# DonggeunYu/Text2Speech

Measured on AMD Instinct MI355X. Metric: WaveGlow forward audio samples/sec (batch 8x16000 per GPU), higher is better.
Workload: dtype bf16x3 (split-bf16 products, f32 accumulate); 1 GPU; WaveGlow forward, batch 8 x 16000 samples per GPU, 12 flows, n_group 8, WN 8 layers x 512 channels (reference waveglow/config.json); per_gpu_batch=8, segment_length=16000, mode=forward, parallelism=replicas, no collective

## Files before the change

### include/t2s_hip.h

```cpp
#ifndef T2S_HIP_H
#define T2S_HIP_H
#include <stddef.h>
#ifdef __cplusplus
extern "C" {
#endif

#define T2S_OK 0
#define T2S_EINVAL (-1)
#define T2S_EHIP (-2)

#define T2S_PERM_NONE 0
#define T2S_PERM_GATE 1
#define T2S_PERM_PAIR8 2
#define T2S_ACT_NONE 0
#define T2S_ACT_RELU 1
#define T2S_ACT_TANH 2

int t2s_abi_version(void);
int t2s_operand_format(void);
int t2s_sizeof_taco_decoder(void);
int t2s_sizeof_taco_bptt(void);
const char* t2s_error_string(int code);
const char* t2s_last_hip_error(void);

int t2s_plane_rows(int L, int halo);
int t2s_padded_rows(int rows);

int t2s_pack_conv_weight(const float* v, const float* g, int g_is_scale, const float* bias_in, int O, int Cin, int Kt,
                         int perm, int C_gate, int row_off, int Mpad, int koff, int Cin_pad, void* A_hi, void* A_lo,
                         float* bias_out, int bias_accumulate, void* stream);

typedef struct t2s_pack_job {
    const float *v, *g, *bias_in, *bias_in2;
    void *A_hi, *A_lo;
    float* bias_out;
    long row_start;
    long O, Cin, Kt, perm, C_gate, Mpad, koff, Cin_pad, row_off, g_is_scale;
    float* scale_out;
} t2s_pack_job;
int t2s_pack_conv_weight_table(const t2s_pack_job* jobs, int n_jobs, long total_groups, void* stream);

int t2s_weightnorm_small(const float* v, const float* g, int O, int K, float* w, void* stream);

int t2s_wg_upsample_squeeze(const float* mel, const float* W, const float* bias, int B, int n_mel, int frames,
                            int ksize, int stride, int n_group, int L, int Lp, int halo, void* S_hi, void* S_lo,
                            void* stream);

int t2s_wg_audio_squeeze(float* audio, float* z, int B, int T, int n_group, int L, int unsqueeze, void* stream);

int t2s_wg_convinv(float* z, const float* W, int B, int n_group, int c_off, int n_rem, int L, void* stream);

int t2s_small_logdet_inv(const float* W, int n, float scale, float* logdet_out, float* inv_out, void* stream);

typedef struct t2s_small_mat_job { const float* W; float* logdet_out; float* inv_out; long n; } t2s_small_mat_job;
int t2s_small_logdet_inv_batch(const t2s_small_mat_job* jobs, int n_jobs, float scale, void* stream);
int t2s_small_logdet_inv_batch_host(const t2s_small_mat_job* host_jobs, int n_jobs, float scale, void* stream);

int t2s_wg_start(const float* z, const float* w, const float* bias, int B, int n_group, int c_off, int n_half, int C,
                 int L, int Lp, int halo, void* X_hi, void* X_lo, void* stream);

int t2s_wg_in_cond_gate(const void* A_hi, const void* A_lo, const float* bias, const void* X_hi, const void* X_lo,
                        const void* S_hi, const void* S_lo, void* acts_hi, void* acts_lo, int B, int C, int n_cond,
                        int taps, int dilation, int L, int Lp, int halo, int Mpad, void* stream);

int t2s_wg_res_skip(const void* A_hi, const void* A_lo, const float* bias, const void* acts_hi, const void* acts_lo,
                    void* X_hi, void* X_lo, float* skip, int B, int C, int n_res, int skip_init, int L, int Lp,
                    int halo, int Mpad, void* stream);

int t2s_wg_end_affine(const float* skip, const float* w_end, const float* b_end, float* z, float* log_s,
                      float* wn_out, int B, int n_group, int c_off, int n_half, int C, int L, int Lp, int halo, int reverse, void* stream);

typedef struct t2s_endfold_job {
    const float *w_end, *v_skip, *scale, *b_skip;
    void* fold_A;
    float* bes;
    long nj, C;
} t2s_endfold_job;
int t2s_wg_endfold_weights(const t2s_endfold_job* jobs, int n_jobs, int C, void* stream);
int t2s_wg_gate_tile_rows(int B, int C, int L);
int t2s_wg_gate_fold_slots(int B, int C, int L);
int t2s_wg_in_cond_gate_fold(const void* A_hi, const void* A_lo, const float* bias, const void* X_hi, const void* X_lo,
                             const void* S_hi, const void* S_lo, void* acts_hi, void* acts_lo, const void* fold_A,
                             float* fold_acc, int fold_init, int B, int C, int n_cond, int taps, int dilation, int L,
                             int Lp, int halo, int Mpad, void* stream);
int t2s_wg_upsample_basis(const float* W, const float* bias, int n_mel, int ksize, int stride, int n_group, int Lp, int halo,
                          void* U_hi, void* U_lo, void* stream);
int t2s_wg_compose_cond(const float* tmp, const float* bias_in, int rows, int Mpad, int P, int K2, long ld, void* A2_hi,
                        void* A2_lo, float* bias_out, void* stream);
int t2s_wg_melwin_planes(const float* mel, int B, int n_mel, int frames, int nlag, int Fp, void* M_hi, void* M_lo, void* stream);
int t2s_wg_in_melwin_gate_fold(const void* A_hi, const void* A_lo, const void* A2_hi, const void* A2_lo, const float* bias,
                               const void* X_hi, const void* X_lo, const void* M_hi, const void* M_lo, void* acts_hi,
                               void* acts_lo, const void* fold_A, float* fold_acc, int fold_init, int B, int C, int K2,
                               int taps, int dilation, int L, int Lp, int halo, int Mpad, int P, int Fp, void* stream);
int t2s_wg_res_only(const void* A_hi, const void* A_lo, const float* bias, const void* acts_hi, const void* acts_lo,
                    void* X_hi, void* X_lo, int B, int C, int L, int Lp, int halo, int Mpad, int pair8, void* stream);
int t2s_wg_end_fold_affine(const float* fold_acc, int nslots, const float* bes, int n_layers, const float* b_end,
                           float* z, float* log_s, float* wn_out, int B, int n_group, int c_off, int n_half, int L, int reverse,
                           void* stream);

int t2s_conv_bias_act(const void* A_hi, const void* A_lo, const float* bias, const void* X_hi, const void* X_lo,
                      void* O_hi, void* O_lo, float* out_f32, int f32_channel_last, int B, int Cin, int Cout, int taps,
                      int dilation, int act, int L, int Lp, int halo, int Mpad, void* stream);


int t2s_gemv(const float* W1, int ld1, int k1, const float* W2, int ld2, int k2, const float* x1, int n1, long sx1,
             const float* x2, int n2, long sx2, const float* x3, int n3, long sx3, const float* bias1,
             const float* bias2, float* y, long sy_item, long sy_row, int rows, int items, int act,
             const unsigned char* mask, long smask_item, float mask_scale, void* stream);

int t2s_transpose(const float* in, float* out, int R, int C, void* stream);

int t2s_embed_planes(const long* ids, const float* emb, int B, int T, int E, int V, int Lp, int halo, void* X_hi,
                     void* X_lo, void* stream);
int t2s_f32_to_planes(const float* x, int B, int C, int L, int Lp, int halo, void* X_hi, void* X_lo, void* stream);
int t2s_taco_parse_output(float* mel, float* mel_post, float* gate, const int* lengths, int B, int n_mel, int T, void* stream);
int t2s_zero_plane_rows(void* X_hi, void* X_lo, const int* lengths, int B, int C, int T, int Lp, int halo, void* stream);
int t2s_zero_rows_f32(float* x, const int* lengths, int B, int N, int row, void* stream);
int t2s_bn_fold(const float* gamma, const float* beta, const float* mean, const float* var, const float* conv_bias,
                float eps, int C, float* scale, float* bias_out, void* stream);

int t2s_bn_train(const float* x, const float* gamma, const float* beta, float eps, int act, const unsigned char* mask,
                 float mask_scale, int B, int C, int T, int Lp, int halo, float* mean, float* var, void* O_hi, void* O_lo,
                 float* out_f32, void* stream);

int t2s_bn_running_update(const float* mean, const float* var, float* running_mean, float* running_var,
                          long long* num_batches_tracked, float momentum, long long n, int C, void* stream);
int t2s_zero_fill(void* p, size_t bytes, void* stream);

int t2s_taco_encoder_lstm(const float* gx, const float* whhT_fwd, const float* whhT_rev, const int* lengths, float* out,
                          int B, int T, int H, int T_out, float* gates_save ,
                          float* c_save , void* stream);
int t2s_taco_encoder_lstm_split(const float* gx, const float* whhT_fwd, const float* whhT_rev, const int* lengths, float* out,
                                int B, int T, int H, int T_out, float* gates_save, float* c_save, void* xbuf, unsigned epoch,
                                void* stream);
long t2s_taco_lstm_xbuf_bytes(int B);
int t2s_taco_encoder_lstm_bwd(const float* d_out, const float* out, const float* gates_save, const float* c_save,
                              const float* whh_fwd, const float* whh_rev, const int* lengths, float* dgx, float* hprev,
                              int B, int T, int H, int T_out, void* stream);
int t2s_taco_encoder_lstm_bwd_split(const float* d_out, const float* out, const float* gates_save, const float* c_save,
                                    const float* whh_fwd, const float* whh_rev, const int* lengths, float* dgx, float* hprev,
                                    int B, int T, int H, int T_out, void* xbuf, unsigned epoch, void* stream);
int t2s_rows_to_planes(const float* x, int B, int T, int C, int Lp, int halo, void* X_hi, void* X_lo, void* stream);
int t2s_embedding_grad(const long* ids, const void* D_hi, const void* D_lo, int B, int T, int E, int V, int Lp, int halo,
                       float* d_emb, void* stream);

int t2s_bernoulli_mask(unsigned char* mask, size_t n, unsigned long long seed, unsigned long long offset, float keep_prob,
                       void* stream);

typedef struct t2s_taco_decoder {
    int B, T_in, n_mel, prenet_dim, enc_dim, att_rnn_dim, dec_rnn_dim, att_dim, loc_filters, loc_kernel;
    int T_cap;
    int teacher_forced;
    int mask_steps;
    const float *att_w_ih, *att_w_hh, *att_b_ih, *att_b_hh;
    const float *dec_w_ih, *dec_w_hh, *dec_b_ih, *dec_b_hh;
    const float *w_query, *w_loc_conv, *w_loc_dense, *w_v;
    const float *w_proj, *b_proj;
    const float *w_projpre, *b_projpre;
    const float *w_loc_denseT;
    const float *w_pre2;
    const float *memory, *pmem;
    const int *mem_lengths;
    const float *pre_all;
    const unsigned char *prenet_masks;
    const unsigned char *att_drop, *dec_drop;
    float att_drop_scale, dec_drop_scale;
    float *att_h0, *att_h1, *att_c, *dec_h0, *dec_h1, *dec_c;
    float *att_w, *att_wcum, *ctx, *q, *energies, *pre1, *pre2;
    float *q_part;
    float *mel_gate_out;
    float *align_out;
    float *hc_all;
    float *att_gates_all, *att_c_all;
    float *dec_gates_all, *dec_c_all;
    float *att_h_all;
    float *q_all, *wcum_all;
    float *gate_part;
    const float *w_pre2T;
    float *ploc;
    float *dec_in_part;
    void *att_xbuf;
    void *pace_flag;
} t2s_taco_decoder;

int t2s_taco_decode_steps(const t2s_taco_decoder* d, int step0, int n_steps, void* stream);

int t2s_taco_attention(const float* h_att, const float* memory, const float* pmem, const int* lengths, float* w, float* w_cum,
                       float* ctx, float* q_scratch, float* e_scratch, const float* w_query, const float* w_loc_conv,
                       const float* w_loc_dense, const float* w_loc_denseT, const float* w_v, int B, int T, int att_rnn,
                       int att_dim, int enc_dim, int loc_filters, int loc_kernel, void* stream);

int t2s_taco_stop_check(const float* mel_gate_out, int B, int n_mel, int T_cap, int step0, int n, float threshold,
                        int* stop_step, void* stream);


int t2s_wg_in_cond_gate_train(const void* A_hi, const void* A_lo, const float* bias, const void* X_hi, const void* X_lo,
                              const void* S_hi, const void* S_lo, void* acts_hi, void* acts_lo, void* T_hi, void* T_lo,
                              void* G_hi, void* G_lo, int B, int C, int n_cond, int taps, int dilation, int L, int Lp,
                              int halo, int Mpad, void* stream);
int t2s_wg_res_skip_train(const void* A_hi, const void* A_lo, const float* bias, const void* acts_hi,
                          const void* acts_lo, const void* R_hi, const void* R_lo, void* X_hi, void* X_lo, float* skip,
                          int B, int C, int n_res, int skip_init, int L, int Lp, int halo, int Mpad, void* stream);

int t2s_wg_in_cond_gate_fold_train(const void* A_hi, const void* A_lo, const float* bias, const void* X_hi, const void* X_lo,
                                   const void* S_hi, const void* S_lo, void* acts_hi, void* acts_lo, void* G_hi, void* G_lo,
                                   int act_bchunks, const void* fold_A, float* fold_acc, int fold_init, int B, int C, int n_cond,
                                   int taps, int dilation, int L, int Lp, int halo, int Mpad, void* stream);
int t2s_wg_res_only_train(const void* A_hi, const void* A_lo, const float* bias, const void* acts_hi, const void* acts_lo,
                          int act_bchunks, const void* R_hi, const void* R_lo, void* X_hi, void* X_lo, int B, int C, int L, int Lp,
                          int halo, int Mpad, int pair8, void* stream);
int t2s_wg_skip_sum(const void* A_hi, const void* A_lo, const float* bias, const void* acts_hi, const void* acts_lo,
                    int n_k_chunks, int act_bchunks, float* skip, int B, int C, int L, int Lp, int halo, int Mpad, void* stream);

int t2s_wg_bwd_gate_dgrad(const void* A_hi, const void* A_lo, const float* zero_bias, const void* DX_hi,
                          const void* DX_lo, const void* DS_hi, const void* DS_lo, const void* acts_hi, const void* acts_lo,
                          const void* G_hi, const void* G_lo, int tg_bchunks, void* DP_hi, void* DP_lo, int dp_bchunks, int B, int C,
                          int L, int Lp, int halo, int Mpad, int pair8, void* stream);

int t2s_conv_accumulate(const void* A_hi, const void* A_lo, const float* zero_bias, const void* X_hi, const void* X_lo,
                        int x_bchunks, void* O_hi, void* O_lo, int B, int Cin, int Cout, int taps, int dilation, int init, int L, int Lp,
                        int halo, int Mpad, int pair8, void* stream);

int t2s_wgrad_gemm(const void* A_hi, const void* A_lo, const void* X_hi, const void* X_lo, const float* zero_bias,
                   float* out, int B, int M, int N, int Mpad, int Npad, int n_tchunks, int k0, int k1, int ksplit,
                   void* stream);
int t2s_wgrad_gemm_flat(const void* A_hi, const void* A_lo, const void* X_hi, const void* X_lo, const float* zero_bias,
                        float* out, int B, int M, int N, int Mpad, int Npad, int n_tchunks, int k0, int k1, int nsplit,
                        void* stream);

typedef struct t2s_wgrad_chunk {
    const void* hi;
    const void* lo;
    long bstride;
} t2s_wgrad_chunk;
int t2s_wgrad_cl(const t2s_wgrad_chunk* a_chunks, int n_a_chunks, const t2s_wgrad_chunk* b_chunks, int n_b_chunks, float* out,
                 int B, int M, int N, int ldp, int k0, int k1, int nsplit, int bias_cols, void* stream);

int t2s_plane_transpose(const void* src_hi, const void* src_lo, int B, int src_chunks, int n_chunks, int Lp, int shift,
                        void* dst_hi, void* dst_lo, int Npad, int n_off, void* stream);
int t2s_tm_ones_row(void* dst_hi, void* dst_lo, int B, int Lp, int halo, int L, int Npad, int n_row, void* stream);
int t2s_pack_transposed(const float* v, const float* scale, int O, int Cin, int Kt, int flip, int O_pad, int Mpad,
                        int koff, void* A_hi, void* A_lo, int pair8, void* stream);
int t2s_wg_bwd_pair8_ok(int B, int rows, int L);
int t2s_weightnorm_scale(const float* v, const float* g, int O, int K, float* scale, void* stream);
int t2s_wn_backward(const float* P, int nsplit, int Prows, int Pcols, int row_off, int col_off, int tap_stride,
                    int col_bias, int n_bias_cols, const float* v, const float* g, int O, int Cin, int Kt, float* dv, float* dg,
                    float* db, int db_accum, void* stream);
int t2s_wg_affine_backward(float* z, float* dz, const float* wn_out, const float* g_log_s, int g_log_s_scalar, float* d_out, int B,
                           int n_group, int c_off, int n_half, int L, void* stream);
long t2s_small_wgrad_scratch(int B, int chunks);
int t2s_small_wgrad(const void* P_hi, const void* P_lo, const float* P_f32, const float* Q, float* out, float* rowsum,
                    float* scratch, int B, int chunks, int Lp, int halo, int L, int R, int J, int Jtot, int q_off, int out_transposed,
                    void* stream);
int t2s_rows_sum(const float* Q, int B, int Jtot, int q_off, int J, int L, float* out, void* stream);
int t2s_wg_start_dgrad(const void* X_hi, const void* X_lo, const float* w, float* dz, int B, int n_group, int c_off,
                       int n_half, int C, int L, int Lp, int halo, void* stream);
int t2s_wg_convinv_wgrad(const float* dz, const float* zin, const float* Winv, const float* gscale_ptr, float gmul,
                         int B, int n_group, int c_off, int n, int L, float* dW, void* stream);
int t2s_wg_upsample_wgrad(const void* D_hi, const void* D_lo, const float* mel, int B, int n_mel, int frames, int ksize,
                          int stride, int n_group, int L, int Lp, int halo, float* dW, float* db, void* stream);

typedef struct t2s_adam_job {
    float* p; const float* g; float* m; float* v;
    long n;
    long blk_start;
} t2s_adam_job;
int t2s_adam_table(const t2s_adam_job* jobs, int n_jobs, long total_blocks, float lr, float beta1, float beta2,
                   float eps, int step, float gscale, float weight_decay, void* stream);

int t2s_rows_to_tm(const float* x, long ld, int items, int items_pad, int shift, int C, void* dst_hi, void* dst_lo,
                   int Npad, int n_off, void* stream);
int t2s_rows_to_tm_batched(const float* x, long ld, long x_bstride, int items, int items_pad, int shift, int C, void* dst_hi,
                           void* dst_lo, long dst_bstride, int Npad, int n_off, int nb, void* stream);
int t2s_lstm_cell_bwd(const float* dh1, long s1, const float* dh2, long s2, const float* dh3, long s3,
                      const unsigned char* drop_mask, float drop_scale, const float* gates, const float* c_new,
                      const float* c_prev, float* dc_carry, float* dgates, int B, int H, void* stream);
int t2s_relu_drop_bwd(const float* dy, const float* y, float scale, size_t n, float* dz, void* stream);

typedef struct t2s_att_bwd {
    const float *dctx1; long sc1; const float *dctx2; long sc2; const float *dctx3; long sc3;
    const float *w_cur; long s_wcur;
    const float *w_prev, *wc_prev; long s_wprev, s_wcprev;
    const float *q, *pmem, *memory; const int *lengths;
    const float *w_loc_conv, *w_loc_dense, *w_v;
    float *dw_carry, *dwc_carry, *d_q, *d_pmem, *d_memory;
    float *dD_part, *dK_part, *dv_part;
    float *dw_buf, *df_buf, *dq_part;
    float *dctx_out;
    int B, T, att_dim, enc_dim, loc_f, loc_ks;
    const float *ctx; long s_ctx;
    float *dw_carry_out, *dwc_carry_out;
} t2s_att_bwd;
int t2s_taco_att_bwd(const t2s_att_bwd* a, void* stream);

typedef struct t2s_taco_bptt {
    int B, T_in, T_out, T_cap;
    int prenet_dim, enc_dim, att_rnn_dim, dec_rnn_dim, att_dim, loc_filters, loc_kernel;
    const float *W_dT, *W_aT, *w_query, *w_loc_conv, *w_loc_dense, *w_v;
    const float *dec_gates_all, *dec_c_all, *att_gates_all, *att_c_all, *q_all, *wcum_all;
    const float *align;
    const float *pmem, *memory; const int *lengths;
    const unsigned char *att_drop, *dec_drop; float att_drop_scale, dec_drop_scale;
    const float *d_hc;
    float *out_d, *out_a, *dg_d, *dg_a, *dq_all;
    float *dc_d, *dc_a, *dw_c, *dwc_c;
    float *d_pmem, *d_memory;
    float *dD_part, *dK_part, *dv_part, *dw_buf, *df_buf, *dq_part;
    float *dctx_all;
    const float *ctx_all; long s_ctx_step, s_ctx_item;
    float *dw_c2, *dwc_c2;
    void *att_xbuf;
} t2s_taco_bptt;
int t2s_taco_bptt_steps(const t2s_taco_bptt* p, int t_hi, int t_lo, void* stream);

int t2s_taco_loss(const float* mel, const float* post, const float* target, size_t n_mel, const float* gate,
                  const float* gate_target, size_t n_gate, float* d_mel, float* d_post, float* d_gate, void* partial,
                  float* out, void* stream);

int t2s_waveglow_loss(const float* z, size_t n_z, const float* const* log_s, const size_t* n_log_s, int n_flows,
                      const float* log_det, float sigma, float* d_z, void* partial, float* out, void* stream);

typedef struct t2s_bn_bwd_args {
    const float *x, *mean, *var, *gamma, *beta; float eps;
    const float *dout_f32; const void *dout_hi, *dout_lo;
    const unsigned char *mask; float mask_scale; int act;
    float *dgamma, *dbeta; void *dx_hi, *dx_lo;
    int B, C, T, Lp, halo;
} t2s_bn_bwd_args;
int t2s_bn_bwd(const t2s_bn_bwd_args* a, void* partial, void* stream);
int t2s_sum_axis0(const float* in, int n0, int n, float* out, void* stream);
int t2s_add3(const float* a, const float* b, const float* c, size_t n, float* out, void* stream);
int t2s_scale_by_scalar(const float* in, size_t n, const float* scalar, float mul, float* out, void* stream);
int t2s_planes_to_f32(const void* X_hi, const void* X_lo, int B, int C, int L, int Lp, int halo, float* out,
                      int accumulate, void* stream);

int t2s_stft_transform(const float* audio, int B, int T, const float* fwd_basis, int n_fft, int hop, float* xp, long ldp,
                       float* ft, float* mag, float* phase, float* magT, long ld_mt, void* stream);
int t2s_mel_from_mag(const float* magT, long ld_mt, int B, int F, const float* mel_basis_p, int n_mel, float clip, float* mel,
                     void* stream);
int t2s_stft_inverse(const float* mag, const float* phase, int B, int F, int n_fft, int hop, const float* inv_basis_t, long ld_rc,
                     const float* bias, float strength, const float* win_sq, float tiny, float* rc, float* frames, float* out,
                     void* stream);

#ifdef __cplusplus
}
#endif
#endif
```

### text2speech_amd/_lib.py

```python
import ctypes
import os

HERE = os.path.dirname(os.path.abspath(__file__))
LIB_PATH = os.environ.get("T2S_LIB_PATH") or os.path.join(HERE, "libt2s_hip.so")

c_int, c_float, c_vp, c_long = ctypes.c_int, ctypes.c_float, ctypes.c_void_p, ctypes.c_long

SIGNATURES = {
    "t2s_abi_version": [],
    "t2s_operand_format": [],
    "t2s_sizeof_taco_decoder": [],
    "t2s_sizeof_taco_bptt": [],
    "t2s_error_string": [c_int],
    "t2s_last_hip_error": [],
    "t2s_plane_rows": [c_int, c_int],
    "t2s_padded_rows": [c_int],
    "t2s_pack_conv_weight": [c_vp, c_vp, c_int, c_vp, c_int, c_int, c_int, c_int, c_int, c_int, c_int, c_int, c_int,
                             c_vp, c_vp, c_vp, c_int, c_vp],
    "t2s_pack_conv_weight_table": [c_vp, c_int, c_long, c_vp],
    "t2s_weightnorm_small": [c_vp, c_vp, c_int, c_int, c_vp, c_vp],
    "t2s_wg_upsample_squeeze": [c_vp, c_vp, c_vp, c_int, c_int, c_int, c_int, c_int, c_int, c_int, c_int, c_int,
                                c_vp, c_vp, c_vp],
    "t2s_wg_audio_squeeze": [c_vp, c_vp, c_int, c_int, c_int, c_int, c_int, c_vp],
    "t2s_wg_convinv": [c_vp, c_vp, c_int, c_int, c_int, c_int, c_int, c_vp],
    "t2s_small_logdet_inv": [c_vp, c_int, c_float, c_vp, c_vp, c_vp],
    "t2s_small_logdet_inv_batch": [c_vp, c_int, c_float, c_vp],
    "t2s_small_logdet_inv_batch_host": [c_vp, c_int, c_float, c_vp],
    "t2s_wg_start": [c_vp, c_vp, c_vp, c_int, c_int, c_int, c_int, c_int, c_int, c_int, c_int, c_vp, c_vp, c_vp],
    "t2s_wg_in_cond_gate": [c_vp, c_vp, c_vp, c_vp, c_vp, c_vp, c_vp, c_vp, c_vp, c_int, c_int, c_int, c_int, c_int,
                            c_int, c_int, c_int, c_int, c_vp],
    "t2s_wg_res_skip": [c_vp, c_vp, c_vp, c_vp, c_vp, c_vp, c_vp, c_vp, c_int, c_int, c_int, c_int, c_int, c_int,
                        c_int, c_int, c_vp],
    "t2s_wg_endfold_weights": [c_vp, c_int, c_int, c_vp],
    "t2s_wg_in_cond_gate_fold": [c_vp] * 11 + [c_int] * 10 + [c_vp],
    "t2s_wg_gate_fold_slots": [c_int, c_int, c_int],
    "t2s_wg_gate_tile_rows": [c_int, c_int, c_int],
    "t2s_wg_upsample_basis": [c_vp, c_vp] + [c_int] * 6 + [c_vp, c_vp, c_vp],
    "t2s_wg_compose_cond": [c_vp, c_vp] + [c_int] * 4 + [c_long, c_vp, c_vp, c_vp, c_vp],
    "t2s_wg_melwin_planes": [c_vp] + [c_int] * 5 + [c_vp, c_vp, c_vp],
    "t2s_wg_in_melwin_gate_fold": [c_vp] * 13 + [c_int] * 12 + [c_vp],
    "t2s_wg_res_only": [c_vp] * 7 + [c_int] * 7 + [c_vp],
    "t2s_wg_end_fold_affine": [c_vp, c_int, c_vp, c_int, c_vp, c_vp, c_vp, c_vp, c_int, c_int, c_int, c_int, c_int, c_int, c_vp],
    "t2s_wg_end_affine": [c_vp, c_vp, c_vp, c_vp, c_vp, c_vp, c_int, c_int, c_int, c_int, c_int, c_int, c_int, c_int,
                          c_int, c_vp],
    "t2s_conv_bias_act": [c_vp, c_vp, c_vp, c_vp, c_vp, c_vp, c_vp, c_vp, c_int, c_int, c_int, c_int, c_int, c_int, c_int,
                          c_int, c_int, c_int, c_int, c_vp],
    "t2s_gemv": [c_vp, c_int, c_int, c_vp, c_int, c_int, c_vp, c_int, c_long, c_vp, c_int, c_long, c_vp, c_int, c_long,
                 c_vp, c_vp, c_vp, c_long, c_long, c_int, c_int, c_int, c_vp, c_long, c_float, c_vp],
    "t2s_transpose": [c_vp, c_vp, c_int, c_int, c_vp],
    "t2s_embed_planes": [c_vp, c_vp, c_int, c_int, c_int, c_int, c_int, c_int, c_vp, c_vp, c_vp],
    "t2s_f32_to_planes": [c_vp, c_int, c_int, c_int, c_int, c_int, c_vp, c_vp, c_vp],
    "t2s_taco_parse_output": [c_vp, c_vp, c_vp, c_vp, c_int, c_int, c_int, c_vp],
    "t2s_zero_plane_rows": [c_vp, c_vp, c_vp, c_int, c_int, c_int, c_int, c_int, c_vp],
    "t2s_zero_rows_f32": [c_vp, c_vp, c_int, c_int, c_int, c_vp],
    "t2s_bn_fold": [c_vp, c_vp, c_vp, c_vp, c_vp, c_float, c_int, c_vp, c_vp, c_vp],
    "t2s_bn_train": [c_vp, c_vp, c_vp, c_float, c_int, c_vp, c_float, c_int, c_int, c_int, c_int, c_int, c_vp, c_vp, c_vp,
                     c_vp, c_vp, c_vp],
    "t2s_taco_encoder_lstm": [c_vp, c_vp, c_vp, c_vp, c_vp, c_int, c_int, c_int, c_int, c_vp, c_vp, c_vp],
    "t2s_taco_encoder_lstm_bwd": [c_vp] * 9 + [c_int] * 4 + [c_vp],
    "t2s_taco_encoder_lstm_split": [c_vp, c_vp, c_vp, c_vp, c_vp, c_int, c_int, c_int, c_int, c_vp, c_vp, c_vp, ctypes.c_uint, c_vp],
    "t2s_taco_lstm_xbuf_bytes": [c_int],
    "t2s_taco_encoder_lstm_bwd_split": [c_vp] * 9 + [c_int] * 4 + [c_vp, ctypes.c_uint, c_vp],
    "t2s_rows_to_planes": [c_vp, c_int, c_int, c_int, c_int, c_int, c_vp, c_vp, c_vp],
    "t2s_embedding_grad": [c_vp, c_vp, c_vp, c_int, c_int, c_int, c_int, c_int, c_int, c_vp, c_vp],
    "t2s_bn_running_update": [c_vp, c_vp, c_vp, c_vp, c_vp, c_float, ctypes.c_longlong, c_int, c_vp],
    "t2s_zero_fill": [c_vp, ctypes.c_size_t, c_vp],
    "t2s_wg_bwd_pair8_ok": [c_int, c_int, c_int],
    "t2s_taco_attention": [c_vp] * 14 + [c_int] * 7 + [c_vp],
    "t2s_bernoulli_mask": [c_vp, ctypes.c_size_t, ctypes.c_ulonglong, ctypes.c_ulonglong, c_float, c_vp],
    "t2s_taco_decode_steps": [c_vp, c_int, c_int, c_vp],
    "t2s_taco_stop_check": [c_vp, c_int, c_int, c_int, c_int, c_int, c_float, c_vp, c_vp],
    "t2s_rows_to_tm": [c_vp, c_long, c_int, c_int, c_int, c_int, c_vp, c_vp, c_int, c_int, c_vp],
    "t2s_rows_to_tm_batched": [c_vp, c_long, c_long, c_int, c_int, c_int, c_int, c_vp, c_vp, c_long, c_int, c_int, c_int, c_vp],
    "t2s_lstm_cell_bwd": [c_vp, c_long, c_vp, c_long, c_vp, c_long, c_vp, c_float, c_vp, c_vp, c_vp, c_vp, c_vp, c_int, c_int,
                          c_vp],
    "t2s_relu_drop_bwd": [c_vp, c_vp, c_float, ctypes.c_size_t, c_vp, c_vp],
    "t2s_taco_att_bwd": [c_vp, c_vp],
    "t2s_taco_bptt_steps": [c_vp, c_int, c_int, c_vp],
    "t2s_bn_bwd": [c_vp, c_vp, c_vp],
    "t2s_waveglow_loss": [c_vp, ctypes.c_size_t, c_vp, c_vp, c_int, c_vp, c_float, c_vp, c_vp, c_vp, c_vp],
    "t2s_taco_loss": [c_vp, c_vp, c_vp, ctypes.c_size_t, c_vp, c_vp, ctypes.c_size_t, c_vp, c_vp, c_vp, c_vp, c_vp, c_vp],
    "t2s_stft_transform": [c_vp, c_int, c_int, c_vp, c_int, c_int, c_vp, c_long, c_vp, c_vp, c_vp, c_vp, c_long, c_vp],
    "t2s_mel_from_mag": [c_vp, c_long, c_int, c_int, c_vp, c_int, c_float, c_vp, c_vp],
    "t2s_stft_inverse": [c_vp, c_vp, c_int, c_int, c_int, c_int, c_vp, c_long, c_vp, c_float, c_vp, c_float, c_vp, c_vp, c_vp,
                         c_vp],
    "t2s_sum_axis0": [c_vp, c_int, c_int, c_vp, c_vp],
    "t2s_add3": [c_vp, c_vp, c_vp, ctypes.c_size_t, c_vp, c_vp],
    "t2s_scale_by_scalar": [c_vp, ctypes.c_size_t, c_vp, c_float, c_vp, c_vp],
    "t2s_planes_to_f32": [c_vp, c_vp, c_int, c_int, c_int, c_int, c_int, c_vp, c_int, c_vp],
    "t2s_wg_in_cond_gate_train": [c_vp] * 13 + [c_int] * 9 + [c_vp],
    "t2s_wg_res_skip_train": [c_vp] * 10 + [c_int] * 8 + [c_vp],
    "t2s_wg_bwd_gate_dgrad": [c_vp] * 11 + [c_int] + [c_vp] * 2 + [c_int] * 8 + [c_vp],
    "t2s_wg_in_cond_gate_fold_train": [c_vp] * 11 + [c_int] + [c_vp] * 2 + [c_int] * 10 + [c_vp],
    "t2s_wg_res_only_train": [c_vp] * 5 + [c_int] + [c_vp] * 4 + [c_int] * 7 + [c_vp],
    "t2s_wg_skip_sum": [c_vp] * 5 + [c_int] * 2 + [c_vp] + [c_int] * 6 + [c_vp],
    "t2s_conv_accumulate": [c_vp] * 5 + [c_int] + [c_vp] * 2 + [c_int] * 11 + [c_vp],
    "t2s_wgrad_gemm": [c_vp] * 6 + [c_int] * 9 + [c_vp],
    "t2s_wgrad_gemm_flat": [c_vp] * 6 + [c_int] * 9 + [c_vp],
    "t2s_wgrad_cl": [c_vp, c_int, c_vp, c_int, c_vp] + [c_int] * 8 + [c_vp],
    "t2s_plane_transpose": [c_vp, c_vp, c_int, c_int, c_int, c_int, c_int, c_vp, c_vp, c_int, c_int, c_vp],
    "t2s_tm_ones_row": [c_vp, c_vp, c_int, c_int, c_int, c_int, c_int, c_int, c_vp],
    "t2s_pack_transposed": [c_vp, c_vp, c_int, c_int, c_int, c_int, c_int, c_int, c_int, c_vp, c_vp, c_int, c_vp],
    "t2s_weightnorm_scale": [c_vp, c_vp, c_int, c_int, c_vp, c_vp],
    "t2s_wn_backward": [c_vp, c_int, c_int, c_int, c_int, c_int, c_int, c_int, c_int, c_vp, c_vp, c_int, c_int, c_int, c_vp, c_vp,
                        c_vp, c_int, c_vp],
    "t2s_wg_affine_backward": [c_vp, c_vp, c_vp, c_vp, c_int, c_vp, c_int, c_int, c_int, c_int, c_int, c_vp],
    "t2s_small_wgrad_scratch": [c_int, c_int],
    "t2s_small_wgrad": [c_vp, c_vp, c_vp, c_vp, c_vp, c_vp, c_vp, c_int, c_int, c_int, c_int, c_int, c_int, c_int, c_int, c_int,
                        c_int, c_vp],
    "t2s_rows_sum": [c_vp, c_int, c_int, c_int, c_int, c_int, c_vp, c_vp],
    "t2s_wg_start_dgrad": [c_vp, c_vp, c_vp, c_vp, c_int, c_int, c_int, c_int, c_int, c_int, c_int, c_int, c_vp],
    "t2s_wg_convinv_wgrad": [c_vp, c_vp, c_vp, c_vp, c_float, c_int, c_int, c_int, c_int, c_int, c_vp, c_vp],
    "t2s_wg_upsample_wgrad": [c_vp, c_vp, c_vp, c_int, c_int, c_int, c_int, c_int, c_int, c_int, c_int, c_int, c_vp, c_vp,
                              c_vp],
    "t2s_adam_table": [c_vp, c_int, c_long, c_float, c_float, c_float, c_float, c_int, c_float, c_float, c_vp],
}
_RESTYPE = {"t2s_error_string": ctypes.c_char_p, "t2s_last_hip_error": ctypes.c_char_p,
            "t2s_small_wgrad_scratch": ctypes.c_long, "t2s_taco_lstm_xbuf_bytes": ctypes.c_long}


class T2SError(RuntimeError):
    pass


_lib = None


def load():
    global _lib
    if _lib is not None:
        return _lib
    if not os.path.exists(LIB_PATH):
        raise T2SError(
            "libt2s_hip.so not found at %s - build it with `python -m text2speech_amd.build` "
            "(there is no CPU fallback on the product path)" % LIB_PATH)
    lib = ctypes.CDLL(LIB_PATH)
    diagnostic = bool(os.environ.get("T2S_LIB_PATH"))
    for name, argtypes in SIGNATURES.items():
        try:
            fn = getattr(lib, name)
        except AttributeError as e:
            if diagnostic:
                continue
            raise T2SError("libt2s_hip.so does not export %s" % name) from e
        fn.argtypes = argtypes
        fn.restype = _RESTYPE.get(name, c_int)
    _lib = lib
    return lib


def ptr(t):
    if t is None:
        return None
    return c_vp(t.data_ptr())


HOST_TIMES = {}
_HOST_TIMING = bool(os.environ.get("T2S_HOST_TIMING"))


def call(name, *args):
    lib = load()
    if _HOST_TIMING:
        import time
        t0 = time.perf_counter()
        rc = getattr(lib, name)(*args)
        c = HOST_TIMES.setdefault(name, [0, 0.0])
        c[0] += 1
        c[1] += time.perf_counter() - t0
    else:
        try:
            fn = getattr(lib, name)
        except AttributeError as e:
            raise T2SError("%s does not export %s (a diagnostic build older than the entry point?)" % (LIB_PATH, name)) from e
        rc = fn(*args)
    if rc != 0:
        msg = lib.t2s_error_string(rc).decode()
        hip = lib.t2s_last_hip_error().decode()
        raise T2SError("%s failed: %s%s" % (name, msg, (" (" + hip + ")") if hip and rc == -2 else ""))
    return rc


def operand_format():
    return load().t2s_operand_format()


def plane_rows(L, halo):
    return load().t2s_plane_rows(L, halo)


def padded_rows(rows):
    return load().t2s_padded_rows(rows)


def current_stream():
    import torch
    return c_vp(torch.cuda.current_stream().cuda_stream)
```

### text2speech_amd/csrc/t2s_api.hip

```cpp
#include "../../include/t2s_hip.h"
#include "t2s_kernels.h"

#include <stdlib.h>
#include <string.h>

static thread_local char g_hip_err[256] = "";

extern "C" int t2s_internal_fail_hip(int e);
static int fail_hip(hipError_t e) { return t2s_internal_fail_hip((int)e); }
extern "C" int t2s_internal_fail_hip(int ei) {
    hipError_t e = (hipError_t)ei;
    strncpy(g_hip_err, hipGetErrorString(e), sizeof(g_hip_err) - 1);
    g_hip_err[sizeof(g_hip_err) - 1] = 0;
    return T2S_EHIP;
}
#define T2S_CHECK_HIP(expr)                   \
    do {                                      \
        hipError_t _e = (expr);               \
        if (_e != hipSuccess) return fail_hip(_e); \
    } while (0)

static inline bool aligned16(const void* p) { return ((uintptr_t)p & 15) == 0; }
static inline int cdiv(int a, int b) { return (a + b - 1) / b; }

extern "C" {

int t2s_abi_version(void) { return 4; }

int t2s_sizeof_taco_decoder(void) { return (int)sizeof(t2s_taco_decoder); }
int t2s_sizeof_taco_bptt(void) { return (int)sizeof(t2s_taco_bptt); }

int t2s_operand_format(void) {
#ifdef T2S_SPLIT_F16
    return 1;
#else
    return 0;
#endif
}

const char* t2s_error_string(int code) {
    switch (code) {
        case T2S_OK: return "ok";
        case T2S_EINVAL: return "invalid argument";
        case T2S_EHIP: return "HIP runtime error";
        default: return "unknown error";
    }
}
const char* t2s_last_hip_error(void) { return g_hip_err; }

int t2s_plane_rows(int L, int halo) { return cdiv(L, 256) * 256 + 2 * halo; }
int t2s_padded_rows(int rows) { return cdiv(rows, 256) * 256; }

int t2s_pack_conv_weight(const float* v, const float* g, int g_is_scale, const float* bias_in, int O, int Cin, int Kt,
                         int perm, int C_gate, int row_off, int Mpad, int koff, int Cin_pad, void* A_hi, void* A_lo,
                         float* bias_out, int bias_accumulate, void* stream) {
    if (!v || !A_hi || !A_lo || O <= 0 || Cin <= 0 || Kt <= 0) return T2S_EINVAL;
    if (Mpad % 256 || koff % 32 || Cin_pad % 32 || Cin_pad < Cin) return T2S_EINVAL;
    if (perm == T2S_PERM_GATE) {
        if (O != 2 * C_gate || cdiv(C_gate, 128) * 256 > Mpad) return T2S_EINVAL;
    } else if (perm == T2S_PERM_NONE) {
        if (row_off < 0 || row_off + O > Mpad) return T2S_EINVAL;
    } else {
        return T2S_EINVAL;
    }
    PackArgs a;
    a.v = v; a.g = g; a.bias_in = bias_in;
    a.A_hi = (u16*)A_hi; a.A_lo = (u16*)A_lo; a.bias_out = bias_out;
    a.O = O; a.Cin = Cin; a.Kt = Kt; a.perm = perm; a.C_gate = C_gate; a.Mpad = Mpad; a.koff = koff;
    a.Cin_pad = Cin_pad; a.bias_accumulate = bias_accumulate; a.row_off = row_off; a.g_is_scale = g_is_scale;
    T2S_CHECK_HIP(t2s_launch_pack(a, (hipStream_t)stream));
    return T2S_OK;
}

int t2s_pack_conv_weight_table(const t2s_pack_job* jobs, int n_jobs, long total_rows, void* stream) {
    if (!jobs || n_jobs <= 0 || total_rows <= 0 || total_rows > 0x7fffffffL) return T2S_EINVAL;
    static_assert(sizeof(t2s_pack_job) == sizeof(PackJob), "t2s_pack_job layout");
    T2S_CHECK_HIP(t2s_launch_pack_table((const PackJob*)jobs, n_jobs, total_rows, (hipStream_t)stream));
    return T2S_OK;
}

int t2s_weightnorm_small(const float* v, const float* g, int O, int K, float* w, void* stream) {
    if (!v || !w || O <= 0 || K <= 0) return T2S_EINVAL;
    T2S_CHECK_HIP(t2s_launch_weightnorm_small(v, g, O, K, w, (hipStream_t)stream));
    return T2S_OK;
}

int t2s_wg_upsample_squeeze(const float* mel, const float* W, const float* bias, int B, int n_mel, int frames,
                            int ksize, int stride, int n_group, int L, int Lp, int halo, void* S_hi, void* S_lo,
                            void* stream) {
    if (!mel || !W || !bias || !S_hi || !S_lo) return T2S_EINVAL;
    if (B <= 0 || n_mel <= 0 || frames <= 0 || L <= 0 || n_group <= 0 || stride <= 0 || ksize % stride) return T2S_EINVAL;
    if (!aligned16(W) || !aligned16(S_hi) || !aligned16(S_lo)) return T2S_EINVAL;
    if (Lp < t2s_plane_rows(L, halo)) return T2S_EINVAL;
    if ((long)L * n_group > (long)(frames - 1) * stride + ksize) return T2S_EINVAL;
    if (n_group == 8 && (stride % 8 || ksize % 8)) return T2S_EINVAL;
    T2S_CHECK_HIP(t2s_launch_upsample_squeeze(mel, W, bias, B, n_mel, frames, ksize, stride, n_group, L, Lp, halo,
                                              (u16*)S_hi, (u16*)S_lo, (hipStream_t)stream));
    return T2S_OK;
}

int t2s_wg_audio_squeeze(float* audio, float* z, int B, int T, int n_group, int L, int unsqueeze, void* stream) {
    if (!audio || !z || B <= 0 || L <= 0 || n_group <= 0 || (long)L * n_group > T) return T2S_EINVAL;
    T2S_CHECK_HIP(t2s_launch_audio_squeeze(audio, z, B, T, n_group, L, unsqueeze, (hipStream_t)stream));
    return T2S_OK;
}

int t2s_wg_convinv(float* z, const float* W, int B, int n_group, int c_off, int n_rem, int L, void* stream) {
    if (!z || !W || B <= 0 || L <= 0 || n_rem <= 0 || n_rem > 16 || c_off < 0 || c_off + n_rem > n_group) return T2S_EINVAL;
    T2S_CHECK_HIP(t2s_launch_convinv(z, W, B, n_group, c_off, n_rem, L, (hipStream_t)stream));
    return T2S_OK;
}

int t2s_small_logdet_inv(const float* W, int n, float scale, float* logdet_out, float* inv_out, void* stream) {
    if (!W || n <= 0 || n > 16 || (!logdet_out && !inv_out)) return T2S_EINVAL;
    T2S_CHECK_HIP(t2s_launch_small_logdet_inv(W, n, scale, logdet_out, inv_out, (hipStream_t)stream));
    return T2S_OK;
}

int t2s_small_logdet_inv_batch(const t2s_small_mat_job* jobs, int n_jobs, float scale, void* stream) {
    if (!jobs || n_jobs <= 0) return T2S_EINVAL;
    static_assert(sizeof(t2s_small_mat_job) == sizeof(SmallMatJob), "t2s_small_mat_job layout");
    T2S_CHECK_HIP(t2s_launch_small_logdet_batch((const SmallMatJob*)jobs, n_jobs, scale, (hipStream_t)stream));
    return T2S_OK;
}

int t2s_small_logdet_inv_batch_host(const t2s_small_mat_job* host_jobs, int n_jobs, float scale, void* stream) {
    if (!host_jobs || n_jobs <= 0 || n_jobs > 16) return T2S_EINVAL;
    for (int i = 0; i < n_jobs; ++i)
        if (!host_jobs[i].W || host_jobs[i].n <= 0 || host_jobs[i].n > 16) return T2S_EINVAL;
    T2S_CHECK_HIP(t2s_launch_small_logdet_batch_host((const SmallMatJob*)host_jobs, n_jobs, scale, (hipStream_t)stream));
    return T2S_OK;
}

int t2s_wg_start(const float* z, const float* w, const float* bias, int B, int n_group, int c_off, int n_half, int C,
                 int L, int Lp, int halo, void* X_hi, void* X_lo, void* stream) {
    if (!z || !w || !bias || !X_hi || !X_lo) return T2S_EINVAL;
    if (B <= 0 || L <= 0 || C <= 0 || n_half <= 0 || n_half > 8 || c_off < 0 || c_off + n_half > n_group) return T2S_EINVAL;
    if (!aligned16(X_hi) || !aligned16(X_lo) || Lp < t2s_plane_rows(L, halo)) return T2S_EINVAL;
    T2S_CHECK_HIP(t2s_launch_start(z, w, bias, B, n_group, c_off, n_half, C, L, Lp, halo, (u16*)X_hi, (u16*)X_lo,
                                   (hipStream_t)stream));
    return T2S_OK;
}

static int check_planes(const void* a, const void* b) { return a && b && aligned16(a) && aligned16(b); }

int t2s_wg_in_cond_gate(const void* A_hi, const void* A_lo, const float* bias, const void* X_hi, const void* X_lo,
                        const void* S_hi, const void* S_lo, void* acts_hi, void* acts_lo, int B, int C, int n_cond,
                        int taps, int dilation, int L, int Lp, int halo, int Mpad, void* stream) {
    if (!check_planes(A_hi, A_lo) || !check_planes(X_hi, X_lo) || !check_planes(acts_hi, acts_lo) || !bias) return T2S_EINVAL;
    if (n_cond > 0 && !check_planes(S_hi, S_lo)) return T2S_EINVAL;
    if (B <= 0 || L <= 0 || C <= 0 || C % 4 || taps <= 0 || !(taps & 1) || dilation <= 0) return T2S_EINVAL;
    if ((taps / 2) * dilation > halo || Lp != t2s_plane_rows(L, halo)) return T2S_EINVAL;
    if (Mpad % 256 || Mpad < cdiv(C, 128) * 256 || !aligned16(bias)) return T2S_EINVAL;
    ConvGemmArgs a;
    memset(&a, 0, sizeof(a));
    a.A_hi = (const u16*)A_hi; a.A_lo = (const u16*)A_lo;
    a.X_hi = (const u16*)X_hi; a.X_lo = (const u16*)X_lo;
    a.S_hi = (const u16*)S_hi; a.S_lo = (const u16*)S_lo;
    a.bias = bias; a.O_hi = (u16*)acts_hi; a.O_lo = (u16*)acts_lo;
    a.xc = cdiv(C, 32); a.sc = cdiv(n_cond, 32); a.oc = cdiv(C, 32);
    a.taps = taps; a.dil = dilation;
    a.nk_x = taps * a.xc; a.nk = a.nk_x + a.sc;
    a.Mpad = Mpad; a.Lp = Lp; a.halo = halo; a.L = L; a.B = B;
    a.n_mtiles = cdiv(C, 128); a.n_ttiles = cdiv(L, 256);
    a.C = C;
    T2S_CHECK_HIP(t2s_launch_conv_gemm(a, EPI_GATE, (hipStream_t)stream));
    return T2S_OK;
}

int t2s_wg_res_skip(const void* A_hi, const void* A_lo, const float* bias, const void* acts_hi, const void* acts_lo,
                    void* X_hi, void* X_lo, float* skip, int B, int C, int n_res, int skip_init, int L, int Lp,
                    int halo, int Mpad, void* stream) {
    if (!check_planes(A_hi, A_lo) || !check_planes(acts_hi, acts_lo) || !bias || !skip || !aligned16(skip)) return T2S_EINVAL;
    if (n_res > 0 && !check_planes(X_hi, X_lo)) return T2S_EINVAL;
    if (B <= 0 || L <= 0 || C <= 0 || C % 4 || (n_res != 0 && n_res != C)) return T2S_EINVAL;
    if (Lp != t2s_plane_rows(L, halo) || Mpad % 256 || Mpad < n_res + C || !aligned16(bias)) return T2S_EINVAL;
    ConvGemmArgs a;
    memset(&a, 0, sizeof(a));
    a.A_hi = (const u16*)A_hi; a.A_lo = (const u16*)A_lo;
    a.X_hi = (const u16*)acts_hi; a.X_lo = (const u16*)acts_lo;
    a.bias = bias; a.O_hi = (u16*)X_hi; a.O_lo = (u16*)X_lo; a.skip = skip;
    a.xc = cdiv(C, 32); a.sc = 0; a.oc = cdiv(C, 32);
    a.taps = 1; a.dil = 1;
    a.nk_x = a.xc; a.nk = a.xc;
    a.Mpad = Mpad; a.Lp = Lp; a.halo = halo; a.L = L; a.B = B;
    a.n_mtiles = cdiv(n_res + C, 256); a.n_ttiles = cdiv(L, 256);
    a.C = C; a.n_res = n_res; a.skip_init = skip_init;
    T2S_CHECK_HIP(t2s_launch_conv_gemm(a, EPI_RESSKIP, (hipStream_t)stream));
    return T2S_OK;
}

int t2s_wg_endfold_weights(const t2s_endfold_job* jobs, int n_jobs, int C, void* stream) {
    if (!jobs || n_jobs <= 0 || C <= 0 || (size_t)8 * C * sizeof(float) > 60 * 1024) return T2S_EINVAL;
    static_assert(sizeof(t2s_endfold_job) == sizeof(EndFoldJob), "t2s_endfold_job layout");
    T2S_CHECK_HIP(t2s_launch_endfold_weights((const EndFoldJob*)jobs, n_jobs, C, (hipStream_t)stream));
    return T2S_OK;
}

static int gate_tile_rows(int B, int C, int L) {
    const long wg256 = (long)cdiv(C, 128) * cdiv(L, 256) * B;
    return (wg256 <= 128 && C % 64 == 0) ? 128 : 256;
}

int t2s_wg_gate_tile_rows(int B, int C, int L) {
    if (B <= 0 || C <= 0 || L <= 0) return T2S_EINVAL;
    return gate_tile_rows(B, C, L);
}

int t2s_wg_gate_fold_slots(int B, int C, int L) {
    if (B <= 0 || C <= 0 || L <= 0) return T2S_EINVAL;
    return gate_tile_rows(B, C, L) == 128 ? 2 * cdiv(C, 64) : 2 * cdiv(C, 128);
}

int t2s_wg_in_cond_gate_fold(const void* A_hi, const void* A_lo, const float* bias, const void* X_hi, const void* X_lo,
                             const void* S_hi, const void* S_lo, void* acts_hi, void* acts_lo, const void* fold_A,
                             float* fold_acc, int fold_init, int B, int C, int n_cond, int taps, int dilation, int L,
                             int Lp, int halo, int Mpad, void* stream) {
    if (!check_planes(A_hi, A_lo) || !check_planes(X_hi, X_lo) || !check_planes(acts_hi, acts_lo) || !bias) return T2S_EINVAL;
    if (!fold_A || !fold_acc || !aligned16(fold_A) || C % 16) return T2S_EINVAL;
    if (n_cond > 0 && !check_planes(S_hi, S_lo)) return T2S_EINVAL;
    if (B <= 0 || L <= 0 || C <= 0 || C % 4 || taps <= 0 || !(taps & 1) || dilation <= 0) return T2S_EINVAL;
    if ((taps / 2) * dilation > halo || Lp != t2s_plane_rows(L, halo)) return T2S_EINVAL;
    if (Mpad % 256 || Mpad < cdiv(C, 128) * 256 || !aligned16(bias)) return T2S_EINVAL;
    ConvGemmArgs a;
    memset(&a, 0, sizeof(a));
    a.A_hi = (const u16*)A_hi; a.A_lo = (const u16*)A_lo;
    a.X_hi = (const u16*)X_hi; a.X_lo = (const u16*)X_lo;
    a.S_hi = (const u16*)S_hi; a.S_lo = (const u16*)S_lo;
    a.bias = bias; a.O_hi = (u16*)acts_hi; a.O_lo = (u16*)acts_lo;
    a.fold_A = (const u16*)fold_A; a.fold_acc = fold_acc; a.fold_init = fold_init;
    a.xc = cdiv(C, 32); a.sc = cdiv(n_cond, 32); a.oc = cdiv(C, 32);
    a.taps = taps; a.dil = dilation;
    a.nk_x = taps * a.xc; a.nk = a.nk_x + a.sc;
    a.Mpad = Mpad; a.Lp = Lp; a.halo = halo; a.L = L; a.B = B;
    const int rows = gate_tile_rows(B, C, L);
    a.n_mtiles = cdiv(C, rows / 2); a.n_ttiles = cdiv(L, 256);
    a.C = C;
    T2S_CHECK_HIP(t2s_launch_conv_gemm(a, EPI_GATE, (hipStream_t)stream, rows));
    return T2S_OK;
}

int t2s_wg_upsample_basis(const float* W, const float* bias, int n_mel, int ksize, int stride, int n_group, int Lp, int halo,
                          void* U_hi, void* U_lo, void* stream) {
    if (!W || !bias || !check_planes(U_hi, U_lo)) return T2S_EINVAL;
    if (n_mel <= 0 || n_group <= 0 || stride <= 0 || ksize <= 0 || ksize % stride || stride % n_group) return T2S_EINVAL;
    const int ncols = (stride / n_group) * (ksize / stride) * n_mel + 1;
    if (halo < 0 || Lp != t2s_plane_rows(ncols, halo)) return T2S_EINVAL;
    T2S_CHECK_HIP(t2s_launch_upbasis_planes(W, bias, n_mel, ksize, stride, n_group, Lp, halo, (u16*)U_hi, (u16*)U_lo,
                                            (hipStream_t)stream));
    return T2S_OK;
}

int t2s_wg_compose_cond(const float* tmp, const float* bias_in, int rows, int Mpad, int P, int K2, long ld, void* A2_hi,
                        void* A2_lo, float* bias_out, void* stream) {
    if (!tmp || !bias_in || !bias_out || !check_planes(A2_hi, A2_lo)) return T2S_EINVAL;
    if (rows <= 0 || Mpad % 256 || rows > Mpad || P <= 0 || K2 <= 0 || K2 % 32 || ld < (long)P * K2 + 1) return T2S_EINVAL;
    T2S_CHECK_HIP(t2s_launch_compose_pack(tmp, bias_in, rows, Mpad, P, K2, (int)ld, (u16*)A2_hi, (u16*)A2_lo, bias_out,
                                          (hipStream_t)stream));
    return T2S_OK;
}

int t2s_wg_melwin_planes(const float* mel, int B, int n_mel, int frames, int nlag, int Fp, void* M_hi, void* M_lo, void* stream) {
    if (!mel || !check_planes(M_hi, M_lo)) return T2S_EINVAL;
    if (B <= 0 || n_mel <= 0 || frames <= 0 || nlag <= 0 || Fp < frames) return T2S_EINVAL;
    T2S_CHECK_HIP(t2s_launch_melwin_planes(mel, B, n_mel, frames, nlag, Fp, (u16*)M_hi, (u16*)M_lo, (hipStream_t)stream));
    return T2S_OK;
}

int t2s_wg_in_melwin_gate_fold(const void* A_hi, const void* A_lo, const void* A2_hi, const void* A2_lo, const float* bias,
                               const void* X_hi, const void* X_lo, const void* M_hi, const void* M_lo, void* acts_hi,
                               void* acts_lo, const void* fold_A, float* fold_acc, int fold_init, int B, int C, int K2,
                               int taps, int dilation, int L, int Lp, int halo, int Mpad, int P, int Fp, void* stream) {
    if (!check_planes(A_hi, A_lo) || !check_planes(A2_hi, A2_lo) || !check_planes(X_hi, X_lo) || !check_planes(M_hi, M_lo) ||
        !check_planes(acts_hi, acts_lo) || !bias)
        return T2S_EINVAL;
    if (!fold_A || !fold_acc || !aligned16(fold_A) || C % 16) return T2S_EINVAL;
    if (B <= 0 || L <= 0 || C <= 0 || C % 4 || taps <= 0 || !(taps & 1) || dilation <= 0 || K2 <= 0 || K2 % 32) return T2S_EINVAL;
    if ((taps / 2) * dilation > halo || Lp != t2s_plane_rows(L, halo)) return T2S_EINVAL;
    if (Mpad % 256 || Mpad < cdiv(C, 128) * 256 || !aligned16(bias) || P <= 0) return T2S_EINVAL;
    const int F = cdiv(L, P);
    if (Fp < F) return T2S_EINVAL;
    if (gate_tile_rows(B, C, L) != 256) return T2S_EINVAL;
    ConvGemmArgs a;
    memset(&a, 0, sizeof(a));
    a.A_hi = (const u16*)A_hi; a.A_lo = (const u16*)A_lo;
    a.A2_hi = (const u16*)A2_hi; a.A2_lo = (const u16*)A2_lo;
    a.X_hi = (const u16*)X_hi; a.X_lo = (const u16*)X_lo;
    a.S_hi = (const u16*)M_hi; a.S_lo = (const u16*)M_lo;
    a.bias = bias; a.O_hi = (u16*)acts_hi; a.O_lo = (u16*)acts_lo;
    a.fold_A = (const u16*)fold_A; a.fold_acc = fold_acc; a.fold_init = fold_init;
    a.xc = cdiv(C, 32); a.sc = K2 / 32; a.oc = cdiv(C, 32);
    a.taps = taps; a.dil = dilation;
    a.nk_x = taps * a.xc; a.nk = a.nk_x + a.sc;
    a.Mpad = Mpad; a.Lp = Lp; a.halo = halo; a.L = L; a.B = B;
    a.n_mtiles = cdiv(C, 128); a.n_ttiles = 0;
    a.C = C;
    a.ph_P = P; a.ph_Fp = Fp;
    a.ph_FT = F <= 64 ? 64 : (F <= 128 ? 128 : 256);
    a.ph_bper = 256 / a.ph_FT;
    a.ph_nft = cdiv(F, a.ph_FT);
    T2S_CHECK_HIP(t2s_launch_gate_gemm_pp(a, (hipStream_t)stream));
    return T2S_OK;
}

int t2s_wg_res_only(const void* A_hi, const void* A_lo, const float* bias, const void* acts_hi, const void* acts_lo,
                    void* X_hi, void* X_lo, int B, int C, int L, int Lp, int halo, int Mpad, int pair8, void* stream) {
    if (!check_planes(A_hi, A_lo) || !check_planes(acts_hi, acts_lo) || !check_planes(X_hi, X_lo) || !bias) return T2S_EINVAL;
    if (B <= 0 || L <= 0 || C <= 0 || C % 4 || Lp != t2s_plane_rows(L, halo) || Mpad % 256 || Mpad < C || !aligned16(bias))
        return T2S_EINVAL;
    ConvGemmArgs a;
    memset(&a, 0, sizeof(a));
    a.A_hi = (const u16*)A_hi; a.A_lo = (const u16*)A_lo;
    a.X_hi = (const u16*)acts_hi; a.X_lo = (const u16*)acts_lo;
    a.bias = bias; a.O_hi = (u16*)X_hi; a.O_lo = (u16*)X_lo;
    a.xc = cdiv(C, 32); a.sc = 0; a.oc = cdiv(C, 32);
    a.taps = 1; a.dil = 1; a.nk_x = a.xc; a.nk = a.xc;
    a.Mpad = Mpad; a.Lp = Lp; a.halo = halo; a.L = L; a.B = B;
    a.n_mtiles = cdiv(C, 128); a.n_ttiles = cdiv(L, 256);
    a.C = 0; a.n_res = C;
    if (pair8 && C % 32) return T2S_EINVAL;
    a.pair8 = pair8 ? 1 : 0;
    T2S_CHECK_HIP(t2s_launch_conv_gemm(a, EPI_RESSKIP, (hipStream_t)stream, 128));
    return T2S_OK;
}

int t2s_wg_end_fold_affine(const float* fold_acc, int nslots, const float* bes, int n_layers, const float* b_end,
                           float* z, float* log_s, float* wn_out, int B, int n_group, int c_off, int n_half, int L, int reverse,
                           void* stream) {
    if (!fold_acc || !bes || !b_end || !z || nslots <= 0 || n_layers <= 0) return T2S_EINVAL;
    if (B <= 0 || L <= 0 || n_half <= 0 || n_half > 4 || c_off < 0 || c_off + 2 * n_half > n_group) return T2S_EINVAL;
    T2S_CHECK_HIP(t2s_launch_end_fold_affine(fold_acc, nslots, bes, n_layers, b_end, z, log_s, wn_out, B, n_group, c_off, n_half,
                                             L, reverse, (hipStream_t)stream));
    return T2S_OK;
}

int t2s_wg_end_affine(const float* skip, const float* w_end, const float* b_end, float* z, float* log_s,
                      float* wn_out, int B, int n_group, int c_off, int n_half, int C, int L, int Lp, int halo, int reverse, void* stream) {
    if (!skip || !w_end || !b_end || !z) return T2S_EINVAL;
    if (B <= 0 || L <= 0 || C <= 0 || n_half <= 0 || n_half > 8 || c_off < 0 || c_off + 2 * n_half > n_group) return T2S_EINVAL;
    if (Lp < t2s_plane_rows(L, halo)) return T2S_EINVAL;
    T2S_CHECK_HIP(t2s_launch_end_affine(skip, w_end, b_end, z, log_s, wn_out, B, n_group, c_off, n_half, C, L, Lp, halo,
                                        reverse, (hipStream_t)stream));
    return T2S_OK;
}

int t2s_conv_bias_act(const void* A_hi, const void* A_lo, const float* bias, const void* X_hi, const void* X_lo,
                      void* O_hi, void* O_lo, float* out_f32, int f32_channel_last, int B, int Cin, int Cout, int taps,
                      int dilation, int act, int L, int Lp, int halo, int Mpad, void* stream) {
    if (!check_planes(A_hi, A_lo) || !check_planes(X_hi, X_lo) || !bias || !aligned16(bias)) return T2S_EINVAL;
    if ((O_hi || O_lo) && !check_planes(O_hi, O_lo)) return T2S_EINVAL;
    if (!O_hi && !out_f32) return T2S_EINVAL;
    if (B <= 0 || L <= 0 || Cin <= 0 || Cout <= 0 || Cout % 4 || taps <= 0 || !(taps & 1) || dilation <= 0) return T2S_EINVAL;
    if ((taps / 2) * dilation > halo || Lp != t2s_plane_rows(L, halo) || Mpad % 256 || Mpad < Cout) return T2S_EINVAL;
    if (act < T2S_ACT_NONE || act > T2S_ACT_TANH) return T2S_EINVAL;
    ConvGemmArgs a;
    memset(&a, 0, sizeof(a));
    a.A_hi = (const u16*)A_hi; a.A_lo = (const u16*)A_lo;
    a.X_hi = (const u16*)X_hi; a.X_lo = (const u16*)X_lo;
    a.bias = bias; a.O_hi = (u16*)O_hi; a.O_lo = (u16*)O_lo; a.out_f32 = out_f32;
    a.xc = cdiv(Cin, 32); a.sc = 0; a.oc = cdiv(Cout, 32);
    a.taps = taps; a.dil = dilation;
    a.nk_x = taps * a.xc; a.nk = a.nk_x;
    a.Mpad = Mpad; a.Lp = Lp; a.halo = halo; a.L = L; a.B = B;
    const int rows = (long)cdiv(Cout, 256) * cdiv(L, 256) * B <= 64 ? 128 : 256;
    a.n_mtiles = cdiv(Cout, rows); a.n_ttiles = cdiv(L, 256);
    a.C = Cout; a.act = act; a.f32_cl = f32_channel_last;
    T2S_CHECK_HIP(t2s_launch_conv_gemm(a, EPI_BIAS_ACT, (hipStream_t)stream, rows));
    return T2S_OK;
}

}
```

### text2speech_amd/csrc/t2s_kernels.h

```cpp
#pragma once
#include <hip/hip_runtime.h>
#include <stdint.h>

typedef unsigned short u16;

enum { EPI_GATE = 0, EPI_RESSKIP = 1, EPI_BIAS_ACT = 2, EPI_GATE_BWD = 3 };
enum { ACT_NONE = 0, ACT_RELU = 1, ACT_TANH = 2 };
enum { PERM_NONE = 0, PERM_GATE = 1, PERM_PAIR8 = 2 };

struct ConvGemmArgs {
    const u16* A_hi;
    const u16* A_lo;
    const u16* X_hi;
    const u16* X_lo;
    const u16* S_hi;
    const u16* S_lo;
    const float* bias;
    u16* O_hi;
    u16* O_lo;
    float* skip;
    float* out_f32;
    int nk;
    int nk_x;
    int xc, sc, oc;
    int xbs;
    int taps, dil;
    int Mpad, Lp, halo, L, B;
    int n_mtiles, n_ttiles;
    int C;
    int n_res;
    int skip_init;
    int act;
    int f32_cl;
    u16* T_hi;
    u16* T_lo;
    u16* G_hi;
    u16* G_lo;
    int tc;
    int pair8;
    int res_init;
    const u16* R_hi;
    const u16* R_lo;
    long a_bstride;
    int ksplit;
    int k0, kchunk, kend;
    int kflat;
    const u16* fold_A;
    float* fold_acc;
    int fold_init;
    const u16* A2_hi;
    const u16* A2_lo;
    int ph_P;
    int ph_FT;
    int ph_bper;
    int ph_nft;
    int ph_Fp;
};

hipError_t t2s_launch_conv_gemm(const ConvGemmArgs& a, int epi, hipStream_t stream, int mt_rows = 256);
hipError_t t2s_launch_gate_gemm_pp(const ConvGemmArgs& a, hipStream_t stream);
hipError_t t2s_launch_bwd_gemm_pp(const ConvGemmArgs& a, int epi, hipStream_t stream);
bool t2s_pp_shape_ok(const ConvGemmArgs& a);

struct WgradChunk {
    const u16* hi;
    const u16* lo;
    long bstride;
};
struct WgradClArgs {
    const WgradChunk* a_chunks;
    const WgradChunk* b_chunks;
    float* P;
    int M, N, ldp, n_mtiles, n_ntiles;
    int B, k0, k1;
    int nslab, kchunk;
    int bias_cols;
};
hipError_t t2s_launch_wgrad_cl(const WgradClArgs& a, hipStream_t stream);

struct PackArgs {
    const float* v;
    const float* g;
    const float* bias_in;
    u16* A_hi;
    u16* A_lo;
    float* bias_out;
    int O, Cin, Kt;
    int perm, C_gate;
    int Mpad;
    int koff;
    int Cin_pad;
    int bias_accumulate;
    int row_off;
    int g_is_scale;
};
hipError_t t2s_launch_pack(const PackArgs& a, hipStream_t stream);
struct PackJob {
    const float* v; const float* g; const float* bias_in; const float* bias_in2;
    u16* A_hi; u16* A_lo; float* bias_out;
    long row_start;
    long O, Cin, Kt, perm, C_gate, Mpad, koff, Cin_pad, row_off, g_is_scale;
    float* scale_out;
};
hipError_t t2s_launch_pack_table(const PackJob* jobs, int n_jobs, long total_rows, hipStream_t stream);
hipError_t t2s_launch_weightnorm_small(const float* v, const float* g, int O, int K, float* w, hipStream_t stream);

hipError_t t2s_launch_upbasis_planes(const float* W, const float* bias, int n_mel, int ksize, int stride, int n_group, int Lp,
                                     int halo, u16* U_hi, u16* U_lo, hipStream_t stream);
hipError_t t2s_launch_compose_pack(const float* tmp, const float* bias_in, int rows, int Mpad, int P, int K2, int ld, u16* A2_hi,
                                   u16* A2_lo, float* bias_out, hipStream_t stream);
hipError_t t2s_launch_melwin_planes(const float* mel, int B, int n_mel, int frames, int nlag, int Fp, u16* S_hi, u16* S_lo,
                                    hipStream_t stream);
hipError_t t2s_launch_upsample_squeeze(const float* mel, const float* W, const float* bias, int B, int n_mel,
                                       int frames, int ksize, int stride, int n_group, int L, int Lp, int halo,
                                       u16* S_hi, u16* S_lo, hipStream_t stream);
hipError_t t2s_launch_audio_squeeze(const float* audio, float* z, int B, int T, int n_group, int L, int unsqueeze,
                                    hipStream_t stream);
hipError_t t2s_launch_convinv(float* z, const float* W, int B, int n_group, int c_off, int n_rem, int L,
                              hipStream_t stream);
struct SmallMatJob { const float* W; float* logdet_out; float* inv_out; long n; };
hipError_t t2s_launch_small_logdet_batch(const SmallMatJob* jobs, int n_jobs, float scale, hipStream_t stream);
hipError_t t2s_launch_small_logdet_batch_host(const SmallMatJob* host_jobs, int n_jobs, float scale, hipStream_t stream);
hipError_t t2s_launch_small_logdet_inv(const float* W, int n, float scale, float* logdet_out, float* inv_out,
                                       hipStream_t stream);
hipError_t t2s_launch_start(const float* z, const float* w, const float* bias, int B, int n_group, int c_off,
                            int n_half, int C, int L, int Lp, int halo, u16* X_hi, u16* X_lo, hipStream_t stream);
struct EndFoldJob {
    const float* w_end;
    const float* v_skip;
    const float* scale;
    const float* b_skip;
    u16* fold_A;
    float* bes;
    long nj, C;
};
hipError_t t2s_launch_endfold_weights(const EndFoldJob* jobs, int n_jobs, int C, hipStream_t stream);
hipError_t t2s_launch_end_fold_affine(const float* fold_acc, int nslots, const float* bes, int n_layers,
                                      const float* b_end, float* z, float* log_s, float* wn_out, int B, int n_group, int c_off,
                                      int n_half, int L, int reverse, hipStream_t stream);
hipError_t t2s_launch_end_affine(const float* skip, const float* w_end, const float* b_end, float* z, float* log_s,
                                 float* wn_out, int B, int n_group, int c_off, int n_half, int C, int L, int Lp, int halo,
                                 int reverse, hipStream_t stream);
```

### text2speech_amd/csrc/waveglow_ops.hip

```cpp
#include "t2s_common.h"
#include "t2s_kernels.h"

#include <string.h>

static __device__ __forceinline__ void pack_row(const float* __restrict__ vrow, const float* g, int g_is_scale, int o,
                                                 int Cin, int Kt, int perm, int C_gate, int row_off, int Mpad, int koff,
                                                 int Cin_pad, u16* A_hi, u16* A_lo, const float* bias_in,
                                                 const float* bias_in2, float* bias_out, int bias_accumulate,
                                                 float* scale_out = nullptr) {
    __shared__ float red[4];
    const int tid = threadIdx.x;
    const int n = Cin * Kt;
    float scale = 1.0f;
    if (g && g_is_scale) {
        scale = g[o];
    } else if (g) {
        float ss = 0.f;
        for (int i = tid; i < n; i += 256) {
            const float x = vrow[i];
            ss += x * x;
        }
        ss = wave_sum(ss);
        if ((tid & 63) == 0) red[tid >> 6] = ss;
        __syncthreads();
        ss = red[0] + red[1] + red[2] + red[3];
        scale = g[o] / sqrtf(ss);
    }
    if (scale_out && tid == 0) scale_out[o] = scale;
    int p;
    if (perm == PERM_GATE) {
        const int gate = o >= C_gate;
        const int ch = gate ? o - C_gate : o;
        p = (ch >> 7) * 256 + ((ch >> 6) & 1) * 128 + (((ch >> 4) & 3) * 2 + gate) * 16 + (ch & 15);
    } else {
        p = o + row_off;
    }
    const int half = (Cin + 1) >> 1;
    for (int i = tid; i < half * Kt; i += 256) {
        const int tap = i / half;
        const int c = (i - tap * half) * 2;
        const float w0 = vrow[c * Kt + tap] * scale;
        const float w1 = (c + 1 < Cin) ? vrow[(c + 1) * Kt + tap] * scale : 0.f;
        const int k = koff + tap * Cin_pad + c;
        const size_t idx = ((size_t)(k >> 5) * Mpad + p) * 32 + (k & 31);
        u16 h0, l0, h1, l1;
        split_bf16(w0, h0, l0);
        split_bf16(w1, h1, l1);
        *(uint32_t*)(A_hi + idx) = h0 | ((uint32_t)h1 << 16);
        *(uint32_t*)(A_lo + idx) = l0 | ((uint32_t)l1 << 16);
    }
    if (tid == 0 && bias_out) {
        float bi = bias_in ? bias_in[o] : 0.f;
        if (bias_in2) bi += bias_in2[o];
        bias_out[p] = bias_accumulate ? bias_out[p] + bi : bi;
    }
}

__global__ __launch_bounds__(256) void pack_kernel(const PackArgs a) {
    const int o = blockIdx.x;
    pack_row(a.v + (size_t)o * a.Cin * a.Kt, a.g, a.g_is_scale, o, a.Cin, a.Kt, a.perm, a.C_gate, a.row_off, a.Mpad,
             a.koff, a.Cin_pad, a.A_hi, a.A_lo, a.bias_in, nullptr, a.bias_out, a.bias_accumulate);
}

static __device__ __forceinline__ int pack_dst_row(const PackJob& j, int o) {
    if (j.perm == PERM_GATE) {
        const int gate = o >= (int)j.C_gate;
        const int ch = gate ? o - (int)j.C_gate : o;
        return (ch >> 7) * 256 + ((ch >> 6) & 1) * 128 + (((ch >> 4) & 3) * 2 + gate) * 16 + (ch & 15);
    }
    if (j.perm == PERM_PAIR8 && o < (int)j.C_gate) {
        const int w = o & 31;
        return (o & ~31) + ((w >> 2) & 1) * 16 + (w >> 3) * 4 + (w & 3) + (int)j.row_off;
    }
    return o + (int)j.row_off;
}
static __device__ __forceinline__ void pack_store2(const PackJob& j, int k, int p, float w0, float w1) {
    const size_t idx = ((size_t)(k >> 5) * (int)j.Mpad + p) * 32 + (k & 31);
    u16 h0, l0, h1, l1;
    split_bf16(w0, h0, l0);
    split_bf16(w1, h1, l1);
    *(uint32_t*)(j.A_hi + idx) = h0 | ((uint32_t)h1 << 16);
    *(uint32_t*)(j.A_lo + idx) = l0 | ((uint32_t)l1 << 16);
}
static __device__ __forceinline__ float sum16(float v) {
    v += __shfl_xor(v, 1, 64); v += __shfl_xor(v, 2, 64); v += __shfl_xor(v, 4, 64); v += __shfl_xor(v, 8, 64);
    return v;
}
#define PACK_MAX_CHUNKS 20
template <int KT>
static __device__ __forceinline__ void pack_rows_regs(const PackJob& j, int o0) {
    const int tid = threadIdx.x, r = tid >> 4, cp = tid & 15;
    const int O = (int)j.O, Cin = (int)j.Cin, Cin_pad = (int)j.Cin_pad, koff = (int)j.koff;
    const int o = o0 + r;
    const bool row_ok = o < O;
    const int n = Cin * KT;
    const int nchunk = (Cin + 31) >> 5;
    const float* vrow = j.v + (size_t)(row_ok ? o : 0) * n;
    float x[PACK_MAX_CHUNKS][2 * KT];
    float ss = 0.f;
#pragma unroll
    for (int cc = 0; cc < PACK_MAX_CHUNKS; ++cc) {
        const int c = cc * 32 + cp * 2;
#pragma unroll
        for (int e = 0; e < 2 * KT; ++e) {
            const int ce = c + e / KT;
            x[cc][e] = (cc < nchunk && row_ok && ce < Cin) ? vrow[c * KT + e] : 0.f;
            ss += x[cc][e] * x[cc][e];
        }
    }
    float scale = 1.0f;
    if (j.g) {
        if (j.g_is_scale) scale = row_ok ? j.g[o] : 1.f;
        else {
            ss = sum16(ss);
            scale = row_ok ? j.g[o] / sqrtf(ss) : 1.f;
        }
    }
    if (!row_ok) return;
    const int p = pack_dst_row(j, o);
    if (cp == 0) {
        if (j.scale_out) j.scale_out[o] = scale;
        if (j.bias_out) {
            float bi = j.bias_in ? j.bias_in[o] : 0.f;
            if (j.bias_in2) bi += j.bias_in2[o];
            j.bias_out[p] = bi;
        }
    }
#pragma unroll
    for (int cc = 0; cc < PACK_MAX_CHUNKS; ++cc) {
        if (cc < nchunk) {
            const int c = cc * 32 + cp * 2;
#pragma unroll
            for (int tap = 0; tap < KT; ++tap)
                pack_store2(j, koff + tap * Cin_pad + c, p, x[cc][tap] * scale, x[cc][KT + tap] * scale);
        }
    }
}

static __device__ __forceinline__ void pack_rows_two_pass(const PackJob& j, int o0, float* s_scale) {
    const int tid = threadIdx.x, lane = tid & 63, wave = tid >> 6;
    const int O = (int)j.O, Cin = (int)j.Cin, Kt = (int)j.Kt, Cin_pad = (int)j.Cin_pad, koff = (int)j.koff;
    const int n = Cin * Kt;
#pragma unroll
    for (int rr = 0; rr < 4; ++rr) {
        const int r = wave * 4 + rr, o = o0 + r;
        float scale = 1.0f;
        if (o < O && j.g) {
            if (j.g_is_scale) {
                scale = j.g[o];
            } else {
                const float* vrow = j.v + (size_t)o * n;
                float ss = 0.f;
                for (int i = lane; i < n; i += 64) {
                    const float x = vrow[i];
                    ss += x * x;
                }
                ss = wave_sum(ss);
                scale = j.g[o] / sqrtf(ss);
            }
        }
        if (lane == 0) {
            s_scale[r] = scale;
            if (o < O) {
                if (j.scale_out) j.scale_out[o] = scale;
                if (j.bias_out) {
                    float bi = j.bias_in ? j.bias_in[o] : 0.f;
                    if (j.bias_in2) bi += j.bias_in2[o];
                    j.bias_out[pack_dst_row(j, o)] = bi;
                }
            }
        }
    }
    __syncthreads();
    const int r = tid >> 4, cp = tid & 15;
    const int o = o0 + r;
    if (o >= O) return;
    const int p = pack_dst_row(j, o);
    const float scale = s_scale[r];
    const float* vrow = j.v + (size_t)o * n;
    const int nchunk = (Cin + 31) >> 5;
    for (int cc = 0; cc < nchunk; ++cc) {
        const int c = cc * 32 + cp * 2;
        for (int tap = 0; tap < Kt; ++tap) {
            const float w0 = c < Cin ? vrow[c * Kt + tap] * scale : 0.f;
            const float w1 = c + 1 < Cin ? vrow[(c + 1) * Kt + tap] * scale : 0.f;
            pack_store2(j, koff + tap * Cin_pad + c, p, w0, w1);
        }
    }
}

__global__ __launch_bounds__(256) void pack_table_kernel(const PackJob* __restrict__ jobs, int n_jobs) {
    __shared__ float s_scale[16];
    const long blk = blockIdx.x;
    int lo = 0, hi = n_jobs - 1;
    while (lo < hi) {
        const int mid = (lo + hi + 1) >> 1;
        if (jobs[mid].row_start <= blk) lo = mid; else hi = mid - 1;
    }
    const PackJob j = jobs[lo];
    const int o0 = (int)(blk - j.row_start) * 16;
    const int nchunk = ((int)j.Cin + 31) >> 5;
    if (nchunk <= PACK_MAX_CHUNKS && !((int)j.Cin & 1) && j.Kt == 3) pack_rows_regs<3>(j, o0);
    else if (nchunk <= PACK_MAX_CHUNKS && !((int)j.Cin & 1) && j.Kt == 1) pack_rows_regs<1>(j, o0);
    else pack_rows_two_pass(j, o0, s_scale);
}
hipError_t t2s_launch_pack_table(const PackJob* jobs, int n_jobs, long total_groups, hipStream_t stream) {
    hipLaunchKernelGGL(pack_table_kernel, dim3((unsigned)total_groups), dim3(256), 0, stream, jobs, n_jobs);
    return hipGetLastError();
}

hipError_t t2s_launch_pack(const PackArgs& a, hipStream_t stream) {
    hipLaunchKernelGGL(pack_kernel, dim3(a.O), dim3(256), 0, stream, a);
    return hipGetLastError();
}

__global__ void weightnorm_small_kernel(const float* v, const float* g, int O, int K, float* w) {
    const int o = blockIdx.x * blockDim.x + threadIdx.x;
    if (o >= O) return;
    float ss = 0.f;
    for (int k = 0; k < K; ++k) ss += v[o * K + k] * v[o * K + k];
    const float s = g ? g[o] / sqrtf(ss) : 1.f;
    for (int k = 0; k < K; ++k) w[o * K + k] = v[o * K + k] * s;
}
hipError_t t2s_launch_weightnorm_small(const float* v, const float* g, int O, int K, float* w, hipStream_t stream) {
    hipLaunchKernelGGL(weightnorm_small_kernel, dim3((O + 255) / 256), dim3(256), 0, stream, v, g, O, K, w);
    return hipGetLastError();
}

template <int BB>
__global__ __launch_bounds__(256) void upsample_squeeze_kernel(const float* __restrict__ mel, const float* __restrict__ W,
                                                               const float* __restrict__ bias, int B, int M, int F,
                                                               int ksize, int stride, int G, int L, int Lp, int halo,
                                                               u16* S_hi, u16* S_lo) {
    const int tid = threadIdx.x;
    const int q = tid & 3;
    const int t = blockIdx.x * 64 + (tid >> 2);
    const int chunk = blockIdx.y;
    const int b0 = blockIdx.z * BB;
    const int c8 = chunk * 32 + q * 8;
    const int nchan = M * G;
    if (t >= L || c8 >= nchan) return;
    float acc[BB][8];
#pragma unroll
    for (int bb = 0; bb < BB; ++bb)
#pragma unroll
        for (int j = 0; j < 8; ++j) acc[bb][j] = 0.f;
    const int nf = ksize / stride;
    if (G == 8) {
        const int co = c8 >> 3;
        const int s0 = 8 * t;
        const int fhi = s0 / stride;
        const int kbase = s0 - fhi * stride;
        for (int ci = 0; ci < M; ++ci) {
            const float* wrow = W + ((size_t)ci * M + co) * ksize + kbase;
            for (int i = 0; i < nf; ++i) {
                const int f = fhi - i;
                if (f < 0 || f >= F) continue;
                const f32x4 w0 = *(const f32x4*)(wrow + i * stride);
                const f32x4 w1 = *(const f32x4*)(wrow + i * stride + 4);
#pragma unroll
                for (int bb = 0; bb < BB; ++bb) {
                    if (b0 + bb >= B) break;
                    const float m = mel[((size_t)(b0 + bb) * M + ci) * F + f];
#pragma unroll
                    for (int j = 0; j < 4; ++j) {
                        acc[bb][j] += m * w0[j];
                        acc[bb][4 + j] += m * w1[j];
                    }
                }
            }
        }
#pragma unroll
        for (int bb = 0; bb < BB; ++bb)
#pragma unroll
            for (int j = 0; j < 8; ++j) acc[bb][j] += bias[co];
    } else {
        for (int j = 0; j < 8; ++j) {
            const int cidx = c8 + j;
            if (cidx >= nchan) break;
            const int co = cidx / G, g = cidx - co * G;
            const int s = G * t + g;
            const int fhi = s / stride;
            for (int ci = 0; ci < M; ++ci)
                for (int i = 0; i < nf; ++i) {
                    const int f = fhi - i;
                    if (f < 0 || f >= F) continue;
                    const float w = W[((size_t)ci * M + co) * ksize + (s - f * stride)];
                    for (int bb = 0; bb < BB; ++bb)
                        if (b0 + bb < B) acc[bb][j] += mel[((size_t)(b0 + bb) * M + ci) * F + f] * w;
                }
            for (int bb = 0; bb < BB; ++bb) acc[bb][j] += bias[co];
        }
    }
    const int nchunks = (nchan + 31) / 32;
#pragma unroll
    for (int bb = 0; bb < BB; ++bb) {
        if (b0 + bb >= B) break;
        const size_t row = ((size_t)(b0 + bb) * nchunks + chunk) * Lp + halo + t;
        u16 hi[8], lo[8];
#pragma unroll
        for (int j = 0; j < 8; ++j) {
            const float v = (c8 + j < nchan) ? acc[bb][j] : 0.f;
            split_bf16(v, hi[j], lo[j]);
        }
        uint4 ph, pl;
        ph.x = hi[0] | ((uint32_t)hi[1] << 16); ph.y = hi[2] | ((uint32_t)hi[3] << 16);
        ph.z = hi[4] | ((uint32_t)hi[5] << 16); ph.w = hi[6] | ((uint32_t)hi[7] << 16);
        pl.x = lo[0] | ((uint32_t)lo[1] << 16); pl.y = lo[2] | ((uint32_t)lo[3] << 16);
        pl.z = lo[4] | ((uint32_t)lo[5] << 16); pl.w = lo[6] | ((uint32_t)lo[7] << 16);
        *(uint4*)(S_hi + row * 32 + q * 8) = ph;
        *(uint4*)(S_lo + row * 32 + q * 8) = pl;
    }
}

typedef float f32x4_up __attribute__((ext_vector_type(4)));
template <int NT, int KB>
__global__ __launch_bounds__(256) void upsample_mfma_kernel(const float* __restrict__ mel, const float* __restrict__ W,
                                                            const float* __restrict__ bias, int B, int M, int F, int ksize,
                                                            int stride, int L, int Lp, int halo, int tiles_per_b, int n_ctiles,
                                                            int n_pairs, int nz, u16* S_hi, u16* S_lo) {
    const int lane = threadIdx.x & 63;
    const int wave = threadIdx.x >> 6;
    const int r = lane & 15, q = lane >> 4;
    const int xcd = blockIdx.x & 7, slot = blockIdx.x >> 3;
    const int pair = (slot / nz) * 8 + xcd;
    if (pair >= n_pairs) return;
    const int npb = stride >> 6;
    const int p0 = ((pair % npb) * 4 + wave) * 16;
    const int chunk = pair / npb;
    const int ct0 = (slot % nz) * NT;
    const float* wa = W + (size_t)(chunk * 4) * ksize + (size_t)q * stride + p0 + r;
    const size_t wa_step = (size_t)M * ksize;
    const float* mb[NT];
    bool mv[NT];
#pragma unroll
    for (int n = 0; n < NT; ++n) {
        const int ct = ct0 + n;
        const int b = ct / tiles_per_b;
        const int f = (ct - b * tiles_per_b) * 16 + r - q;
        mv[n] = ct < n_ctiles && b < B && f >= 0 && f < F;
        mb[n] = mel + ((size_t)(mv[n] ? b : 0) * M) * F + (mv[n] ? f : 0);
    }
    f32x4_up acc[4][NT];
#pragma unroll
    for (int o = 0; o < 4; ++o)
#pragma unroll
        for (int n = 0; n < NT; ++n) acc[o][n] = (f32x4_up){0.f, 0.f, 0.f, 0.f};
    float a_cur[KB][4], b_cur[KB][NT], a_nxt[KB][4], b_nxt[KB][NT];
#pragma unroll
    for (int kk = 0; kk < KB; ++kk) {
#pragma unroll
        for (int o = 0; o < 4; ++o) a_cur[kk][o] = wa[(size_t)kk * wa_step + (size_t)o * ksize];
#pragma unroll
        for (int n = 0; n < NT; ++n) b_cur[kk][n] = mv[n] ? mb[n][(size_t)kk * F] : 0.f;
    }
    for (int ci = 0; ci < M; ci += KB) {
        const int cn = ci + KB < M ? ci + KB : ci;
#pragma unroll
        for (int kk = 0; kk < KB; ++kk) {
#pragma unroll
            for (int o = 0; o < 4; ++o) a_nxt[kk][o] = wa[(size_t)(cn + kk) * wa_step + (size_t)o * ksize];
#pragma unroll
            for (int n = 0; n < NT; ++n) b_nxt[kk][n] = mv[n] ? mb[n][(size_t)(cn + kk) * F] : 0.f;
        }
#pragma unroll
        for (int kk = 0; kk < KB; ++kk)
#pragma unroll
            for (int o = 0; o < 4; ++o)
#pragma unroll
                for (int n = 0; n < NT; ++n)
                    acc[o][n] = __builtin_amdgcn_mfma_f32_16x16x4f32(a_cur[kk][o], b_cur[kk][n], acc[o][n], 0, 0, 0);
#pragma unroll
        for (int kk = 0; kk < KB; ++kk) {
#pragma unroll
            for (int o = 0; o < 4; ++o) a_cur[kk][o] = a_nxt[kk][o];
#pragma unroll
            for (int n = 0; n < NT; ++n) b_cur[kk][n] = b_nxt[kk][n];
        }
    }
    const int nchunks = (M * 8 + 31) / 32;
    const int tpf = stride >> 3;
    const int pq = p0 + 4 * q;
#pragma unroll
    for (int n = 0; n < NT; ++n) {
        const int ct = ct0 + n;
        const int b = ct / tiles_per_b;
        const int f = (ct - b * tiles_per_b) * 16 + r;
        const int t = f * tpf + (pq >> 3);
        if (ct >= n_ctiles || b >= B || t >= L) continue;
        const size_t row = (((size_t)b * nchunks + chunk) * Lp + halo + t) * 32 + (pq & 7);
#pragma unroll
        for (int o = 0; o < 4; ++o) {
            const float bo = bias[chunk * 4 + o];
            u16 hi[4], lo[4];
#pragma unroll
            for (int e = 0; e < 4; ++e) split_bf16(acc[o][n][e] + bo, hi[e], lo[e]);
            uint2 ph, pl;
            ph.x = hi[0] | ((uint32_t)hi[1] << 16); ph.y = hi[2] | ((uint32_t)hi[3] << 16);
            pl.x = lo[0] | ((uint32_t)lo[1] << 16); pl.y = lo[2] | ((uint32_t)lo[3] << 16);
            *(uint2*)(S_hi + row + o * 8) = ph;
            *(uint2*)(S_lo + row + o * 8) = pl;
        }
    }
}

hipError_t t2s_launch_upsample_squeeze(const float* mel, const float* W, const float* bias, int B, int n_mel,
                                       int frames, int ksize, int stride, int n_group, int L, int Lp, int halo,
                                       u16* S_hi, u16* S_lo, hipStream_t stream) {
    const int nchunks = (n_mel * n_group + 31) / 32;
    if (n_group == 8 && ksize == 4 * stride && stride % 64 == 0 && n_mel % 4 == 0) {
        const int nf = (8 * L - 1) / stride + 1;
        const int tiles_per_b = (nf + 15) / 16;
        const int n_ctiles = tiles_per_b * B;
        constexpr int NT = 2;
        const int nz = (n_ctiles + NT - 1) / NT;
        const int n_pairs = (stride / 64) * (n_mel / 4);
        dim3 grid(8 * ((n_pairs + 7) / 8) * nz);
        hipLaunchKernelGGL((upsample_mfma_kernel<NT, 1>), grid, dim3(256), 0, stream, mel, W, bias, B, n_mel, frames, ksize,
                           stride, L, Lp, halo, tiles_per_b, n_ctiles, n_pairs, nz, S_hi, S_lo);
        return hipGetLastError();
    }
    constexpr int BB = 8;
    dim3 grid((L + 63) / 64, nchunks, (B + BB - 1) / BB);
    hipLaunchKernelGGL(upsample_squeeze_kernel<BB>, grid, dim3(256), 0, stream, mel, W, bias, B, n_mel, frames, ksize,
                       stride, n_group, L, Lp, halo, S_hi, S_lo);
    return hipGetLastError();
}

__global__ __launch_bounds__(256) void upbasis_planes_kernel(const float* __restrict__ W, const float* __restrict__ bias, int M,
                                                             int ksize, int stride, int G, int P, int K2, int Lp, int halo,
                                                             u16* U_hi, u16* U_lo) {
    const int q = threadIdx.x & 3;
    const int col = blockIdx.x * 64 + (threadIdx.x >> 2);
    const int chunk = blockIdx.y;
    const int ncols = P * K2 + 1;
    if (col >= ncols) return;
    const int c8 = chunk * 32 + q * 8;
    u16 hi[8], lo[8];
#pragma unroll
    for (int e = 0; e < 8; ++e) {
        const int c = c8 + e;
        float v = 0.f;
        if (c < M * G) {
            const int co = c / G, g = c - co * G;
            if (col == ncols - 1) {
                v = bias[co];
            } else {
                const int phi = col / K2, k = col - phi * K2;
                const int j = k / M, ci = k - j * M;
                v = W[((size_t)ci * M + co) * ksize + (size_t)stride * j + G * phi + g];
            }
        }
        split_bf16(v, hi[e], lo[e]);
    }
    const size_t row = ((size_t)chunk * Lp + halo + col) * 32 + q * 8;
    uint4 ph, pl;
    ph.x = hi[0] | ((uint32_t)hi[1] << 16); ph.y = hi[2] | ((uint32_t)hi[3] << 16);
    ph.z = hi[4] | ((uint32_t)hi[5] << 16); ph.w = hi[6] | ((uint32_t)hi[7] << 16);
    pl.x = lo[0] | ((uint32_t)lo[1] << 16); pl.y = lo[2] | ((uint32_t)lo[3] << 16);
    pl.z = lo[4] | ((uint32_t)lo[5] << 16); pl.w = lo[6] | ((uint32_t)lo[7] << 16);
    *(uint4*)(U_hi + row) = ph;
    *(uint4*)(U_lo + row) = pl;
}
hipError_t t2s_launch_upbasis_planes(const float* W, const float* bias, int n_mel, int ksize, int stride, int n_group, int Lp,
                                     int halo, u16* U_hi, u16* U_lo, hipStream_t stream) {
    const int P = stride / n_group, K2 = (ksize / stride) * n_mel;
    const int ncols = P * K2 + 1;
    dim3 grid((ncols + 63) / 64, (n_mel * n_group + 31) / 32);
    hipLaunchKernelGGL(upbasis_planes_kernel, grid, dim3(256), 0, stream, W, bias, n_mel, ksize, stride, n_group, P, K2, Lp, halo,
                       U_hi, U_lo);
    return hipGetLastError();
}

__global__ __launch_bounds__(256) void compose_pack_kernel(const float* __restrict__ tmp, const float* __restrict__ bias_in,
                                                           int rows, int Mpad, int P, int K2, int ld, u16* A2_hi, u16* A2_lo,
                                                           float* bias_out) {
    const int q = threadIdx.x & 3;
    const int m = blockIdx.x * 64 + (threadIdx.x >> 2);
    const int kc = blockIdx.y, phi = blockIdx.z;
    if (m >= Mpad) return;
    u16 hi[8], lo[8];
#pragma unroll
    for (int e = 0; e < 8; ++e) {
        const int k = kc * 32 + q * 8 + e;
        const float v = (m < rows && k < K2) ? tmp[(size_t)m * ld + (size_t)phi * K2 + k] : 0.f;
        split_bf16(v, hi[e], lo[e]);
    }
    const int mc = (K2 + 31) / 32;
    const size_t o = ((((size_t)phi * mc + kc) * Mpad) + m) * 32 + q * 8;
    uint4 ph, pl;
    ph.x = hi[0] | ((uint32_t)hi[1] << 16); ph.y = hi[2] | ((uint32_t)hi[3] << 16);
    ph.z = hi[4] | ((uint32_t)hi[5] << 16); ph.w = hi[6] | ((uint32_t)hi[7] << 16);
    pl.x = lo[0] | ((uint32_t)lo[1] << 16); pl.y = lo[2] | ((uint32_t)lo[3] << 16);
    pl.z = lo[4] | ((uint32_t)lo[5] << 16); pl.w = lo[6] | ((uint32_t)lo[7] << 16);
    *(uint4*)(A2_hi + o) = ph;
    *(uint4*)(A2_lo + o) = pl;
    if (kc == 0 && phi == 0 && q == 0) bias_out[m] = bias_in[m] + (m < rows ? tmp[(size_t)m * ld + (size_t)P * K2] : 0.f);
}
hipError_t t2s_launch_compose_pack(const float* tmp, const float* bias_in, int rows, int Mpad, int P, int K2, int ld, u16* A2_hi,
                                   u16* A2_lo, float* bias_out, hipStream_t stream) {
    dim3 grid((Mpad + 63) / 64, (K2 + 31) / 32, P);
    hipLaunchKernelGGL(compose_pack_kernel, grid, dim3(256), 0, stream, tmp, bias_in, rows, Mpad, P, K2, ld, A2_hi, A2_lo, bias_out);
    return hipGetLastError();
}

__global__ __launch_bounds__(256) void melwin_planes_kernel(const float* __restrict__ mel, int M, int F, int nlag, int Fp,
                                                            u16* S_hi, u16* S_lo) {
    const int q = threadIdx.x & 3;
    const int f = blockIdx.x * 64 + (threadIdx.x >> 2);
    const int chunk = blockIdx.y, b = blockIdx.z;
    if (f >= Fp) return;
    const int K2 = nlag * M, mc = (K2 + 31) / 32;
    u16 hi[8], lo[8];
#pragma unroll
    for (int e = 0; e < 8; ++e) {
        const int k = chunk * 32 + q * 8 + e;
        float v = 0.f;
        if (k < K2) {
            const int j = k / M, ci = k - j * M;
            const int ff = f - j;
            if (ff >= 0 && ff < F) v = mel[((size_t)b * M + ci) * F + ff];
        }
        split_bf16(v, hi[e], lo[e]);
    }
    const size_t o = (((size_t)b * mc + chunk) * Fp + f) * 32 + q * 8;
    uint4 ph, pl;
    ph.x = hi[0] | ((uint32_t)hi[1] << 16); ph.y = hi[2] | ((uint32_t)hi[3] << 16);
    ph.z = hi[4] | ((uint32_t)hi[5] << 16); ph.w = hi[6] | ((uint32_t)hi[7] << 16);
    pl.x = lo[0] | ((uint32_t)lo[1] << 16); pl.y = lo[2] | ((uint32_t)lo[3] << 16);
    pl.z = lo[4] | ((uint32_t)lo[5] << 16); pl.w = lo[6] | ((uint32_t)lo[7] << 16);
    *(uint4*)(S_hi + o) = ph;
    *(uint4*)(S_lo + o) = pl;
}
hipError_t t2s_launch_melwin_planes(const float* mel, int B, int n_mel, int frames, int nlag, int Fp, u16* S_hi, u16* S_lo,
                                    hipStream_t stream) {
    dim3 grid((Fp + 63) / 64, (nlag * n_mel + 31) / 32, B);
    hipLaunchKernelGGL(melwin_planes_kernel, grid, dim3(256), 0, stream, mel, n_mel, frames, nlag, Fp, S_hi, S_lo);
    return hipGetLastError();
}

__global__ void audio_squeeze_kernel(const float* audio, float* z, int B, int T, int G, int L, int unsq) {
    const int t = blockIdx.x * blockDim.x + threadIdx.x;
    const int b = blockIdx.y;
    if (t >= L) return;
    for (int g = 0; g < G; ++g) {
        if (unsq)
            ((float*)audio)[(size_t)b * T + (size_t)G * t + g] = z[((size_t)b * G + g) * L + t];
        else
            z[((size_t)b * G + g) * L + t] = audio[(size_t)b * T + (size_t)G * t + g];
    }
}
hipError_t t2s_launch_audio_squeeze(const float* audio, float* z, int B, int T, int n_group, int L, int unsqueeze,
                                    hipStream_t stream) {
    hipLaunchKernelGGL(audio_squeeze_kernel, dim3((L + 255) / 256, B), dim3(256), 0, stream, audio, z, B, T, n_group,
                       L, unsqueeze);
    return hipGetLastError();
}

__global__ void convinv_kernel(float* z, const float* __restrict__ W, int G, int c_off, int n, int L) {
    __shared__ float w[16 * 16];
    if (threadIdx.x < n * n) w[threadIdx.x] = W[threadIdx.x];
    __syncthreads();
    const int t = blockIdx.x * blockDim.x + threadIdx.x;
    const int b = blockIdx.y;
    if (t >= L) return;
    float* base = z + ((size_t)b * G + c_off) * L + t;
    float v[16], o[16];
    for (int j = 0; j < n; ++j) v[j] = base[(size_t)j * L];
    for (int i = 0; i < n; ++i) {
        float s = 0.f;
        for (int j = 0; j < n; ++j) s += w[i * n + j] * v[j];
        o[i] = s;
    }
    for (int i = 0; i < n; ++i) base[(size_t)i * L] = o[i];
}
hipError_t t2s_launch_convinv(float* z, const float* W, int B, int n_group, int c_off, int n_rem, int L,
                              hipStream_t stream) {
    hipLaunchKernelGGL(convinv_kernel, dim3((L + 255) / 256, B), dim3(256), 0, stream, z, W, n_group, c_off, n_rem, L);
    return hipGetLastError();
}

__global__ void small_logdet_inv_kernel(const float* W, int n, float scale, float* logdet_out, float* inv_out) {
    __shared__ double a[16][32];
    if (threadIdx.x != 0 || blockIdx.x != 0) return;
    for (int i = 0; i < n; ++i)
        for (int j = 0; j < n; ++j) {
            a[i][j] = W[i * n + j];
            a[i][n + j] = (i == j) ? 1.0 : 0.0;
        }
    double logabs = 0.0;
    int sign = 1;
    for (int c = 0; c < n; ++c) {
        int piv = c;
        double best = fabs(a[c][c]);
        for (int r = c + 1; r < n; ++r)
            if (fabs(a[r][c]) > best) { best = fabs(a[r][c]); piv = r; }
        if (piv != c) {
            for (int j = 0; j < 2 * n; ++j) { double tmp = a[c][j]; a[c][j] = a[piv][j]; a[piv][j] = tmp; }
            sign = -sign;
        }
        const double d = a[c][c];
        if (d < 0) sign = -sign;
        logabs += log(fabs(d));
        const double inv = 1.0 / d;
        for (int j = 0; j < 2 * n; ++j) a[c][j] *= inv;
        for (int r = 0; r < n; ++r) {
            if (r == c) continue;
            const double f = a[r][c];
            if (f == 0.0) continue;
            for (int j = 0; j < 2 * n; ++j) a[r][j] -= f * a[c][j];
        }
    }
    if (logdet_out) *logdet_out = sign > 0 ? (float)(logabs * (double)scale) : __builtin_nanf("");
    if (inv_out)
        for (int i = 0; i < n; ++i)
            for (int j = 0; j < n; ++j) inv_out[i * n + j] = (float)a[i][n + j];
}
static __device__ __forceinline__ void small_logdet_one(const SmallMatJob& j, float scale, double (*a)[32]) {
    const int n = (int)j.n;
    for (int i = 0; i < n; ++i)
        for (int c = 0; c < n; ++c) {
            a[i][c] = j.W[i * n + c];
            a[i][n + c] = (i == c) ? 1.0 : 0.0;
        }
    double logabs = 0.0;
    int sign = 1;
    for (int c = 0; c < n; ++c) {
        int piv = c;
        double best = fabs(a[c][c]);
        for (int r = c + 1; r < n; ++r)
            if (fabs(a[r][c]) > best) { best = fabs(a[r][c]); piv = r; }
        if (piv != c) {
            for (int q = 0; q < 2 * n; ++q) { double tmp = a[c][q]; a[c][q] = a[piv][q]; a[piv][q] = tmp; }
            sign = -sign;
        }
        const double d = a[c][c];
        if (d < 0) sign = -sign;
        logabs += log(fabs(d));
        const double inv = 1.0 / d;
        for (int q = 0; q < 2 * n; ++q) a[c][q] *= inv;
        for (int r = 0; r < n; ++r) {
            if (r == c) continue;
            const double f = a[r][c];
            if (f == 0.0) continue;
            for (int q = 0; q < 2 * n; ++q) a[r][q] -= f * a[c][q];
        }
    }
    if (j.logdet_out) *j.logdet_out = sign > 0 ? (float)(logabs * (double)scale) : __builtin_nanf("");
    if (j.inv_out)
        for (int i = 0; i < n; ++i)
            for (int c = 0; c < n; ++c) j.inv_out[i * n + c] = (float)a[i][n + c];
}
__global__ void small_logdet_batch_kernel(const SmallMatJob* jobs, float scale) {
    __shared__ double a[16][32];
    if (threadIdx.x != 0) return;
    small_logdet_one(jobs[blockIdx.x], scale, a);
}
struct SmallMatJobs16 { SmallMatJob j[16]; };
__global__ void small_logdet_batch_val_kernel(const SmallMatJobs16 jobs, float scale) {
    __shared__ double a[16][32];
    if (threadIdx.x != 0) return;
    small_logdet_one(jobs.j[blockIdx.x], scale, a);
}
hipError_t t2s_launch_small_logdet_batch(const SmallMatJob* jobs, int n_jobs, float scale, hipStream_t stream) {
    hipLaunchKernelGGL(small_logdet_batch_kernel, dim3(n_jobs), dim3(64), 0, stream, jobs, scale);
    return hipGetLastError();
}
hipError_t t2s_launch_small_logdet_batch_host(const SmallMatJob* host_jobs, int n_jobs, float scale, hipStream_t stream) {
    if (n_jobs > 16) return hipErrorInvalidValue;
    SmallMatJobs16 v;
    memset(&v, 0, sizeof(v));
    for (int i = 0; i < n_jobs; ++i) v.j[i] = host_jobs[i];
    hipLaunchKernelGGL(small_logdet_batch_val_kernel, dim3(n_jobs), dim3(64), 0, stream, v, scale);
    return hipGetLastError();
}

hipError_t t2s_launch_small_logdet_inv(const float* W, int n, float scale, float* logdet_out, float* inv_out,
                                       hipStream_t stream) {
    hipLaunchKernelGGL(small_logdet_inv_kernel, dim3(1), dim3(64), 0, stream, W, n, scale, logdet_out, inv_out);
    return hipGetLastError();
}

#define START_TT 8
__global__ __launch_bounds__(256) void start_kernel(const float* __restrict__ z, const float* __restrict__ w,
                                                    const float* __restrict__ bias, int G, int c_off, int nh, int C,
                                                    int L, int Lp, int halo, u16* X_hi, u16* X_lo) {
    const int tid = threadIdx.x;
    const int q = tid & 3;
    const int tbase = blockIdx.x * (64 * START_TT) + (tid >> 2);
    const int chunk = blockIdx.y;
    const int b = blockIdx.z;
    const int c8 = chunk * 32 + q * 8;
    float wv[8][8], bv[8];
#pragma unroll
    for (int e = 0; e < 8; ++e) {
        const int c = c8 + e;
        bv[e] = c < C ? bias[c] : 0.f;
#pragma unroll
        for (int j = 0; j < 8; ++j) wv[e][j] = (c < C && j < nh) ? w[c * nh + j] : 0.f;
    }
    const int nchunks = (C + 31) / 32;
    const size_t row0 = ((size_t)b * nchunks + chunk) * Lp + halo;
#pragma unroll 2
    for (int it = 0; it < START_TT; ++it) {
        const int t = tbase + it * 64;
        if (t >= L) break;
        float a0[8];
#pragma unroll
        for (int j = 0; j < 8; ++j) a0[j] = j < nh ? z[((size_t)b * G + c_off + j) * L + t] : 0.f;
        u16 hi[8], lo[8];
#pragma unroll
        for (int e = 0; e < 8; ++e) {
            float v = bv[e];
#pragma unroll
            for (int j = 0; j < 8; ++j)
                if (j < nh) v += wv[e][j] * a0[j];
            split_bf16(v, hi[e], lo[e]);
        }
        uint4 ph, pl;
        ph.x = hi[0] | ((uint32_t)hi[1] << 16); ph.y = hi[2] | ((uint32_t)hi[3] << 16);
        ph.z = hi[4] | ((uint32_t)hi[5] << 16); ph.w = hi[6] | ((uint32_t)hi[7] << 16);
        pl.x = lo[0] | ((uint32_t)lo[1] << 16); pl.y = lo[2] | ((uint32_t)lo[3] << 16);
        pl.z = lo[4] | ((uint32_t)lo[5] << 16); pl.w = lo[6] | ((uint32_t)lo[7] << 16);
        *(uint4*)(X_hi + (row0 + t) * 32 + q * 8) = ph;
        *(uint4*)(X_lo + (row0 + t) * 32 + q * 8) = pl;
    }
}
hipError_t t2s_launch_start(const float* z, const float* w, const float* bias, int B, int n_group, int c_off,
                            int n_half, int C, int L, int Lp, int halo, u16* X_hi, u16* X_lo, hipStream_t stream) {
    dim3 grid((L + 64 * START_TT - 1) / (64 * START_TT), (C + 31) / 32, B);
    hipLaunchKernelGGL(start_kernel, grid, dim3(256), 0, stream, z, w, bias, n_group, c_off, n_half, C, L, Lp, halo,
                       X_hi, X_lo);
    return hipGetLastError();
}

__global__ __launch_bounds__(256) void end_affine_kernel(const float* __restrict__ skip, const float* __restrict__ w_end,
                                                         const float* __restrict__ b_end, float* z, float* log_s,
                                                         float* wn_out, int G, int c_off, int nh, int C, int L, int Lp,
                                                         int halo, int reverse) {
    const int tid = threadIdx.x;
    const int l32 = tid & 31;
    const int t = blockIdx.x * 8 + (tid >> 5);
    const int b = blockIdx.y;
    const int nj = 2 * nh;
    const int nchunks = (C + 31) / 32;
    float part[16];
#pragma unroll
    for (int j = 0; j < 16; ++j) part[j] = 0.f;
    const bool tv = t < L;
    if (tv) {
        for (int ck = 0; ck < nchunks; ++ck) {
            const int c = ck * 32 + l32;
            if (c < C) {
                const float v = skip[(((size_t)b * nchunks + ck) * Lp + halo + t) * 32 + l32];
#pragma unroll
                for (int j = 0; j < 16; ++j)
                    if (j < nj) part[j] += v * w_end[j * C + c];
            }
        }
    }
#pragma unroll
    for (int j = 0; j < 16; ++j) {
        if (j < nj) {
#pragma unroll
            for (int off = 16; off > 0; off >>= 1) part[j] += __shfl_xor(part[j], off, 64);
        }
    }
    if (tv && l32 < nh) {
        float bb = 0.f, ls = 0.f;
#pragma unroll
        for (int j = 0; j < 16; ++j) {
            if (j == l32) bb = part[j];
            if (j == nh + l32) ls = part[j];
        }
        bb += b_end[l32];
        ls += b_end[nh + l32];
        float* zp = z + ((size_t)b * G + c_off + nh + l32) * L + t;
        const float a1 = *zp;
        *zp = reverse ? (a1 - bb) / expf(ls) : expf(ls) * a1 + bb;
        if (log_s) log_s[((size_t)b * nh + l32) * L + t] = ls;
        if (wn_out) {
            wn_out[((size_t)b * 2 * nh + l32) * L + t] = bb;
            wn_out[((size_t)b * 2 * nh + nh + l32) * L + t] = ls;
        }
    }
}
hipError_t t2s_launch_end_affine(const float* skip, const float* w_end, const float* b_end, float* z, float* log_s,
                                 float* wn_out, int B, int n_group, int c_off, int n_half, int C, int L, int Lp, int halo,
                                 int reverse, hipStream_t stream) {
    hipLaunchKernelGGL(end_affine_kernel, dim3((L + 7) / 8, B), dim3(256), 0, stream, skip, w_end, b_end, z, log_s, wn_out,
                       n_group, c_off, n_half, C, L, Lp, halo, reverse);
    return hipGetLastError();
}

__global__ __launch_bounds__(256) void endfold_weights_kernel(const EndFoldJob* __restrict__ jobs, int C) {
    extern __shared__ float s_ws[];
    __shared__ float red[4];
    const EndFoldJob j = jobs[blockIdx.x];
    const int tid = threadIdx.x;
    const int nj = (int)j.nj;
    for (int i = tid; i < 8 * C; i += 256) {
        const int r = i / C, o = i - r * C;
        s_ws[i] = (r < nj) ? j.w_end[(size_t)r * C + o] * (j.scale ? j.scale[o] : 1.f) : 0.f;
    }
    __syncthreads();
    const int c = blockIdx.y * 256 + tid;
    if (c < C) {
        float acc[8];
#pragma unroll
        for (int r = 0; r < 8; ++r) acc[r] = 0.f;
        for (int o = 0; o < C; ++o) {
            const float v = j.v_skip[(size_t)o * C + c];
#pragma unroll
            for (int r = 0; r < 8; ++r) acc[r] += s_ws[r * C + o] * v;
        }
        const int mt = c >> 7, wr = (c >> 6) & 1, pair = (c >> 5) & 1, half = (c >> 4) & 1, q = (c >> 2) & 3, reg = c & 3;
        u16* base = j.fold_A + ((size_t)((mt * 2 + wr) * 2 + pair) * 2 * 64) * 8;
#pragma unroll
        for (int r = 0; r < 8; ++r) {
            u16 h, l;
            split_bf16(acc[r], h, l);
            const int lane = q * 16 + r;
            base[(size_t)lane * 8 + half * 4 + reg] = h;
            base[(size_t)(64 + lane) * 8 + half * 4 + reg] = l;
        }
    }
    if (blockIdx.y == 0) {
        for (int r = 0; r < 8; ++r) {
            float s = 0.f;
            if (r < nj)
                for (int o = tid; o < C; o += 256) s += j.w_end[(size_t)r * C + o] * j.b_skip[o];
            s = wave_sum(s);
            __syncthreads();
            if ((tid & 63) == 0) red[tid >> 6] = s;
            __syncthreads();
            if (tid == 0) j.bes[r] = red[0] + red[1] + red[2] + red[3];
        }
    }
}
hipError_t t2s_launch_endfold_weights(const EndFoldJob* jobs, int n_jobs, int C, hipStream_t stream) {
    hipLaunchKernelGGL(endfold_weights_kernel, dim3(n_jobs, (C + 255) / 256), dim3(256), (size_t)8 * C * sizeof(float),
                       stream, jobs, C);
    return hipGetLastError();
}

__global__ void end_fold_affine_kernel(const float* __restrict__ fold_acc, int nslots, const float* __restrict__ bes,
                                       int n_layers, const float* __restrict__ b_end, float* z, float* log_s, float* wn_out,
                                       int B, int G, int c_off, int nh, int L, int reverse) {
    const int t = blockIdx.x * blockDim.x + threadIdx.x;
    const int i = blockIdx.y, b = blockIdx.z;
    if (t >= L) return;
    float bb = b_end[i], ls = b_end[nh + i];
    for (int l = 0; l < n_layers; ++l) { bb += bes[l * 8 + i]; ls += bes[l * 8 + nh + i]; }
    for (int s = 0; s < nslots; ++s) {
        bb += fold_acc[(((size_t)s * B + b) * 8 + i) * L + t];
        ls += fold_acc[(((size_t)s * B + b) * 8 + nh + i) * L + t];
    }
    float* zp = z + ((size_t)b * G + c_off + nh + i) * L + t;
    const float a1 = *zp;
    *zp = reverse ? (a1 - bb) / expf(ls) : expf(ls) * a1 + bb;
    if (log_s) log_s[((size_t)b * nh + i) * L + t] = ls;
    if (wn_out) {
        wn_out[((size_t)b * 2 * nh + i) * L + t] = bb;
        wn_out[((size_t)b * 2 * nh + nh + i) * L + t] = ls;
    }
}
hipError_t t2s_launch_end_fold_affine(const float* fold_acc, int nslots, const float* bes, int n_layers,
                                      const float* b_end, float* z, float* log_s, float* wn_out, int B, int n_group, int c_off,
                                      int n_half, int L, int reverse, hipStream_t stream) {
    hipLaunchKernelGGL(end_fold_affine_kernel, dim3((L + 255) / 256, n_half, B), dim3(256), 0, stream, fold_acc, nslots, bes,
                       n_layers, b_end, z, log_s, wn_out, B, n_group, c_off, n_half, L, reverse);
    return hipGetLastError();
}
```

### text2speech_amd/glow.py

```python
import ctypes
import math

import os

import torch
import torch.nn.functional as F

from . import _lib


class _WaveGlowLossFn(torch.autograd.Function):

    @staticmethod
    def forward(ctx, sigma, n_flows, z, *rest):
        log_s = [t.detach().to(torch.float32).contiguous() for t in rest[:n_flows]]
        dets = [t.detach() for t in rest[n_flows:]]
        d0 = dets[0]
        if all(t.dtype == torch.float32 and t.dim() == 0 and t.untyped_storage().data_ptr() == d0.untyped_storage().data_ptr()
               and t.storage_offset() == d0.storage_offset() + k for k, t in enumerate(dets)):
            log_det = d0.as_strided((n_flows,), (1,))
        else:
            log_det = torch.stack([t.to(torch.float32).reshape(()) for t in dets])
        zc = z.detach().to(torch.float32).contiguous()
        dev = zc.device
        d_z = torch.empty_like(zc) if z.requires_grad else None
        partial = torch.empty(256 * 2, dtype=torch.float64, device=dev)
        out = torch.empty(1, dtype=torch.float32, device=dev)
        ptrs = (ctypes.c_void_p * n_flows)(*[t.data_ptr() for t in log_s])
        counts = (ctypes.c_size_t * n_flows)(*[t.numel() for t in log_s])
        _lib.call("t2s_waveglow_loss", _lib.ptr(zc), zc.numel(), ptrs, counts, n_flows, _lib.ptr(log_det), float(sigma),
                  _lib.ptr(d_z), _lib.ptr(partial), _lib.ptr(out), _lib.current_stream())
        ctx.d_z, ctx.n_flows, ctx.inv_n = d_z, n_flows, 1.0 / zc.numel()
        ctx.meta = [(t.shape, t.requires_grad) for t in rest]
        ctx.z_shape = z.shape
        return out.view(())

    @staticmethod
    def backward(ctx, g):
        g32 = g.detach().to(torch.float32).contiguous()
        st = _lib.current_stream()
        gz = None
        if ctx.d_z is not None:
            gz = torch.empty_like(ctx.d_z)
            _lib.call("t2s_scale_by_scalar", _lib.ptr(ctx.d_z), gz.numel(), _lib.ptr(g32), 1.0, _lib.ptr(gz), st)
            gz = gz.view(ctx.z_shape)
        neg = torch.empty(1, dtype=torch.float32, device=g32.device)
        _lib.call("t2s_scale_by_scalar", None, 1, _lib.ptr(g32), -ctx.inv_n, _lib.ptr(neg), st)
        outs = [neg.view(()).expand(shape) if need else None for shape, need in ctx.meta]
        return (None, None, gz, *outs)


class WaveGlowLoss(torch.nn.Module):

    def __init__(self, sigma=1.0):
        super().__init__()
        self.sigma = sigma

    def forward(self, model_output):
        z, log_s_list, log_det_W_list = model_output
        if not z.is_cuda:
            raise _lib.T2SError("WaveGlowLoss (MI355X build) needs tensors in HBM; there is no CPU path")
        if len(log_s_list) > 16 or len(log_s_list) != len(log_det_W_list):
            raise ValueError("WaveGlowLoss: at most 16 flows, one log_det_W per log_s")
        return _WaveGlowLossFn.apply(float(self.sigma), len(log_s_list), z, *log_s_list, *log_det_W_list)


class Invertible1x1Conv(torch.nn.Module):

    def __init__(self, c):
        super().__init__()
        self.conv = torch.nn.Conv1d(c, c, kernel_size=1, stride=1, padding=0, bias=False)
        W = torch.linalg.qr(torch.randn(c, c))[0]
        if torch.det(W) < 0:
            W[:, 0] = -1 * W[:, 0]
        self.conv.weight.data = W.contiguous().view(c, c, 1)

    def forward(self, z, reverse=False):
        if not z.is_cuda:
            raise _lib.T2SError("Invertible1x1Conv (MI355X build) needs tensors in HBM; there is no CPU path")
        B, c, T = z.shape
        st = _lib.current_stream()
        out = z.detach().to(torch.float32).contiguous().clone()
        W = _f32c(self.conv.weight).view(c, c)
        with torch.no_grad():
            if reverse:
                if not hasattr(self, "W_inverse"):
                    Winv = torch.empty(c, c, dtype=torch.float32, device=z.device)
                    _lib.call("t2s_small_logdet_inv", _lib.ptr(W), c, 1.0, None, _lib.ptr(Winv), st)
                    self.W_inverse = Winv.view(c, c, 1)
                Wi = self.W_inverse.detach().to(torch.float32).contiguous()
                _lib.call("t2s_wg_convinv", _lib.ptr(out), _lib.ptr(Wi), B, c, 0, c, T, st)
                return out.to(z.dtype)
            log_det = torch.empty(1, dtype=torch.float32, device=z.device)
            _lib.call("t2s_small_logdet_inv", _lib.ptr(W), c, float(B * T), _lib.ptr(log_det), None, st)
            _lib.call("t2s_wg_convinv", _lib.ptr(out), _lib.ptr(W), B, c, 0, c, T, st)
            return out.to(z.dtype), log_det[0]


class WN(torch.nn.Module):

    def __init__(self, n_in_channels, n_mel_channels, n_layers, n_channels, kernel_size):
        super().__init__()
        assert kernel_size % 2 == 1
        assert n_channels % 2 == 0
        self.n_layers = n_layers
        self.n_channels = n_channels
        self.kernel_size = kernel_size
        self.in_layers = torch.nn.ModuleList()
        self.res_skip_layers = torch.nn.ModuleList()
        self.cond_layers = torch.nn.ModuleList()
        wn = torch.nn.utils.weight_norm
        self.start = wn(torch.nn.Conv1d(n_in_channels, n_channels, 1), name="weight")
        end = torch.nn.Conv1d(n_channels, 2 * n_in_channels, 1)
        end.weight.data.zero_()
        end.bias.data.zero_()
        self.end = end
        for i in range(n_layers):
            dilation = 2 ** i
            padding = (kernel_size * dilation - dilation) // 2
            self.in_layers.append(wn(torch.nn.Conv1d(n_channels, 2 * n_channels, kernel_size,
                                                     dilation=dilation, padding=padding), name="weight"))
            self.cond_layers.append(wn(torch.nn.Conv1d(n_mel_channels, 2 * n_channels, 1), name="weight"))
            rs = 2 * n_channels if i < n_layers - 1 else n_channels
            self.res_skip_layers.append(wn(torch.nn.Conv1d(n_channels, rs, 1), name="weight"))

    def __getstate__(self):
        d = self.__dict__.copy()
        d.pop("_owner", None)
        return d

    def forward(self, forward_input):
        ref = self.__dict__.get("_owner")
        owner = ref() if ref is not None else None
        if owner is None:
            raise _lib.T2SError("WN.forward runs on the engine of the WaveGlow it belongs to; build it through WaveGlow(...)")
        audio, spect = forward_input
        with torch.no_grad():
            return owner._eng().wn_forward(self.__dict__["_flow"], audio, spect)


def _vg(conv):
    if hasattr(conv, "weight_v"):
        return conv.weight_v, conv.weight_g
    return conv.weight, None


def _f32c(t):
    return t.detach().to(torch.float32).contiguous()


class _Engine:

    def __init__(self, model):
        self.m = model
        self.packed = None
        self.packed_key = None
        self.ws = {}
        self.use_fold = True
        self.grad_sync = None
        self.gemm_events = None
        self.gemm_event_stride = 1
        self._gemm_launch_no = 0

    def geom(self):
        m = self.m
        wn0 = m.WN[0]
        C, nl, ks = wn0.n_channels, wn0.n_layers, wn0.kernel_size
        n_cond = m.upsample.out_channels * m.n_group
        halo = -(-((2 ** (nl - 1)) * (ks // 2)) // 32) * 32
        g = dict(C=C, nl=nl, ks=ks, n_cond=n_cond, Cpad=-(-C // 32) * 32, Spad=-(-n_cond // 32) * 32,
                 halo=halo, Mpad1=-(-C // 128) * 256)
        g["nk1"] = ks * g["Cpad"] // 32 + g["Spad"] // 32
        g["nk2"] = g["Cpad"] // 32
        return g

    def pack_weights(self, device, force=True, flow_events=None, res_pair8=False):
        m = self.m
        res_pair8 = bool(res_pair8) and self.geom()["C"] % 32 == 0
        key = tuple(p._version for p in m.parameters()) + (str(device), res_pair8)
        if not force and self.packed is not None and self.packed_key == key:
            return self.packed
        g = self.geom()
        C, nl, ks = g["C"], g["nl"], g["ks"]
        st = _lib.current_stream()
        if self.packed is None or self.packed["device"] != device:
            flows = []
            for k in range(m.n_flows):
                n_half = m.WN[k].start.in_channels
                layers = []
                for i in range(nl):
                    rows2 = 2 * C if i < nl - 1 else C
                    Mpad2 = _lib.padded_rows(rows2)
                    layers.append(dict(
                        A1h=torch.zeros(g["nk1"], g["Mpad1"], 32, dtype=torch.bfloat16, device=device),
                        A1l=torch.zeros(g["nk1"], g["Mpad1"], 32, dtype=torch.bfloat16, device=device),
                        b1=torch.zeros(g["Mpad1"], dtype=torch.float32, device=device),
                        A2h=torch.zeros(g["nk2"], Mpad2, 32, dtype=torch.bfloat16, device=device),
                        A2l=torch.zeros(g["nk2"], Mpad2, 32, dtype=torch.bfloat16, device=device),
                        b2=torch.zeros(Mpad2, dtype=torch.float32, device=device), Mpad2=Mpad2,
                        s_in=torch.empty(2 * C, dtype=torch.float32, device=device),
                        s_cond=torch.empty(2 * C, dtype=torch.float32, device=device),
                        s_rs=torch.empty(rows2, dtype=torch.float32, device=device),
                        fold_A=torch.zeros(-(-C // 128) * 8192, dtype=torch.bfloat16, device=device)))
                flows.append(dict(layers=layers, n_half=n_half, bes=torch.zeros(nl, 8, dtype=torch.float32, device=device),
                                  w_start=torch.empty(C, n_half, dtype=torch.float32, device=device),
                                  w_inv=None))
            self.packed = dict(flows=flows, device=device)
        srcs = []
        specs = []
        for k in range(m.n_flows):
            wn = m.WN[k]
            fl = self.packed["flows"][k]
            for i in range(nl):
                ly = fl["layers"][i]
                v, gg = _vg(wn.in_layers[i])
                vc, gc = _vg(wn.cond_layers[i])
                vr, gr = _vg(wn.res_skip_layers[i])
                t = [_f32c(v), None if gg is None else _f32c(gg), _f32c(wn.in_layers[i].bias), _f32c(wn.cond_layers[i].bias),
                     _f32c(vc), None if gc is None else _f32c(gc),
                     _f32c(vr), None if gr is None else _f32c(gr), _f32c(wn.res_skip_layers[i].bias)]
                srcs += t
                specs.append((t[0], t[1], t[2], t[3], ly["A1h"], ly["A1l"], ly["b1"], 2 * C, C, ks, 1, C, g["Mpad1"], 0, g["Cpad"],
                              ly["s_in"]))
                specs.append((t[4], t[5], None, None, ly["A1h"], ly["A1l"], None, 2 * C, g["n_cond"], 1, 1, C, g["Mpad1"],
                              ks * g["Cpad"], g["Spad"], ly["s_cond"]))
                p8 = res_pair8 and i < nl - 1
                specs.append((t[6], t[7], t[8], None, ly["A2h"], ly["A2l"], ly["b2"], t[6].size(0), C, 1, 2 if p8 else 0,
                              C if p8 else 0, ly["Mpad2"], 0, g["Cpad"], ly["s_rs"]))
        ptr_key = tuple(0 if t is None else t.data_ptr() for t in srcs) + (res_pair8,)
        jpf = 3 * nl
        if self.packed.get("job_key") != ptr_key:
            rows, flow_rows, row_start = [], [], 0
            dp = lambda t: 0 if t is None else t.data_ptr()
            for n, (v, gg, b1, b2, Ah, Al, bo, O, Cin, Kt, perm, Cg, Mpad, koff, Cin_pad, so) in enumerate(specs):
                if n % jpf == 0 and n:
                    flow_rows.append(row_start)
                    row_start = 0
                rows.append([dp(v), dp(gg), dp(b1), dp(b2), dp(Ah), dp(Al), dp(bo), row_start,
                             O, Cin, Kt, perm, Cg, Mpad, koff, Cin_pad, 0, 0, dp(so)])
                row_start += -(-O // 16)
            flow_rows.append(row_start)
            self.packed["jobs"] = torch.tensor(rows, dtype=torch.int64).to(device)
            self.packed["flow_rows"] = flow_rows
            self.packed["job_key"] = ptr_key
        fsrc = []
        for k in range(m.n_flows):
            wn = m.WN[k]
            fl = self.packed["flows"][k]
            w_end = _f32c(wn.end.weight)
            for i in range(nl):
                vr = _f32c(_vg(wn.res_skip_layers[i])[0])
                br = _f32c(wn.res_skip_layers[i].bias)
                r0 = C if i < nl - 1 else 0
                fsrc.append((w_end, vr, br, r0, fl["layers"][i], fl["bes"], i, 2 * fl["n_half"]))
        fkey = tuple((a.data_ptr(), b.data_ptr(), c.data_ptr()) for a, b, c, *_ in fsrc)
        if self.packed.get("fold_key") != fkey:
            rows = []
            for (w_end, vr, br, r0, ly, bes, i, nj) in fsrc:
                rows.append([w_end.data_ptr(), vr.data_ptr() + 4 * r0 * C, ly["s_rs"].data_ptr() + 4 * r0,
                             br.data_ptr() + 4 * r0, ly["fold_A"].data_ptr(), bes.data_ptr() + 4 * 8 * i, nj, C])
            self.packed["fold_jobs"] = torch.tensor(rows, dtype=torch.int64).to(device)
            self.packed["fold_key"] = fkey
        jobs_ptr, fold_ptr = self.packed["jobs"].data_ptr(), self.packed["fold_jobs"].data_ptr()
        starts = []
        for k in range(m.n_flows):
            wn = m.WN[k]
            fl = self.packed["flows"][k]
            _lib.call("t2s_pack_conv_weight_table", _lib.c_vp(jobs_ptr + k * jpf * 19 * 8), jpf, self.packed["flow_rows"][k], st)
            _lib.call("t2s_wg_endfold_weights", _lib.c_vp(fold_ptr + k * nl * 8 * 8), nl, C, st)
            v, gg = _vg(wn.start)
            v, gg = _f32c(v), (None if gg is None else _f32c(gg))
            starts += [v, gg]
            _lib.call("t2s_weightnorm_small", _lib.ptr(v), _lib.ptr(gg), C, fl["n_half"], _lib.ptr(fl["w_start"]), st)
            fl["w_inv"] = None
            if flow_events is not None:
                ev = torch.cuda.Event()
                ev.record()
                flow_events.append(ev)
        keep = srcs + [t for tup in fsrc for t in tup[:3]] + starts
        self.packed_key = key
        self.packed["res_pair8"] = res_pair8
        self._keep = keep
        return self.packed

    def compose_geom(self):
        m, g = self.m, self.geom()
        up = m.upsample
        ksz, stride, G = up.kernel_size[0], up.stride[0], m.n_group
        if os.environ.get("T2S_COND_COMPOSE") != "1" or not self.use_fold:
            return None
        if ksz % stride or stride % G or ((ksz // stride) * up.in_channels) % 32 or g["C"] % 16:
            return None
        return stride // G, ksz // stride, (ksz // stride) * up.in_channels

    def compose_cond(self, device):
        if self.packed.get("compose_key") == self.packed_key:
            return
        m, g = self.m, self.geom()
        P, nlag, K2 = self.compose_geom()
        C, nl, ks = g["C"], g["nl"], g["ks"]
        up = m.upsample
        st = _lib.current_stream()
        ncols = P * K2 + 1
        Lp_u = _lib.plane_rows(ncols, 0)
        sc = g["Spad"] // 32
        bf = dict(dtype=torch.bfloat16, device=device)
        U_h, U_l = torch.zeros(1, sc, Lp_u, 32, **bf), torch.zeros(1, sc, Lp_u, 32, **bf)
        W, bias = _f32c(up.weight), _f32c(up.bias)
        _lib.call("t2s_wg_upsample_basis", _lib.ptr(W), _lib.ptr(bias), up.in_channels, up.kernel_size[0], up.stride[0],
                  m.n_group, Lp_u, 0, _lib.ptr(U_h), _lib.ptr(U_l), st)
        tmp = torch.empty(2 * C, ncols, dtype=torch.float32, device=device)
        zb = torch.zeros(g["Mpad1"], dtype=torch.float32, device=device)
        cond_off = (ks * g["Cpad"] // 32) * g["Mpad1"] * 32 * 2
        mc = K2 // 32
        for k in range(m.n_flows):
            for i in range(nl):
                ly = self.packed["flows"][k]["layers"][i]
                if "Ach" not in ly:
                    ly["Ach"] = torch.zeros(P, mc, g["Mpad1"], 32, **bf)
                    ly["Acl"] = torch.zeros(P, mc, g["Mpad1"], 32, **bf)
                    ly["b1c"] = torch.zeros(g["Mpad1"], dtype=torch.float32, device=device)
                _lib.call("t2s_conv_bias_act", _lib.c_vp(ly["A1h"].data_ptr() + cond_off), _lib.c_vp(ly["A1l"].data_ptr() + cond_off),
                          _lib.ptr(zb), _lib.ptr(U_h), _lib.ptr(U_l), None, None, _lib.ptr(tmp), 0, 1, g["n_cond"], 2 * C, 1, 1, 0,
                          ncols, Lp_u, 0, g["Mpad1"], st)
                _lib.call("t2s_wg_compose_cond", _lib.ptr(tmp), _lib.ptr(ly["b1"]), 2 * C, g["Mpad1"], P, K2, ncols,
                          _lib.ptr(ly["Ach"]), _lib.ptr(ly["Acl"]), _lib.ptr(ly["b1c"]), st)
        self._keep_compose = (U_h, U_l, tmp, zb, W, bias)
        self.packed["compose_key"] = self.packed_key

    def workspace(self, B, L, device):
        key = (B, L, str(device))
        w = self.ws.get(key)
        if w is None:
            g = self.geom()
            Lp = _lib.plane_rows(L, g["halo"])
            bf = dict(dtype=torch.bfloat16, device=device)
            xc, sc = g["Cpad"] // 32, g["Spad"] // 32
            w = dict(Lp=Lp,
                     Xh=torch.zeros(B, xc, Lp, 32, **bf), Xl=torch.zeros(B, xc, Lp, 32, **bf),
                     Ah=torch.zeros(B, xc, Lp, 32, **bf), Al=torch.zeros(B, xc, Lp, 32, **bf),
                     Sh=torch.zeros(B, sc, Lp, 32, **bf), Sl=torch.zeros(B, sc, Lp, 32, **bf),
                     skip=torch.zeros(B, xc, Lp, 32, dtype=torch.float32, device=device),
                     fold_acc=torch.zeros(_lib.load().t2s_wg_gate_fold_slots(B, g["C"], L), B, 8, L, dtype=torch.float32,
                                          device=device))
            self.ws = {key: w}
        return w

    def _check_inputs(self, *tensors):
        for t in tensors:
            if not t.is_cuda:
                raise _lib.T2SError("WaveGlow (MI355X build) needs CUDA/HIP tensors; got a %s tensor - there is no "
                                    "CPU fallback" % t.device)

    def _upsample(self, mel, B, L, w):
        m, g = self.m, self.geom()
        up = m.upsample
        mel32 = _f32c(mel)
        W, bias = _f32c(up.weight), _f32c(up.bias)
        _lib.call("t2s_wg_upsample_squeeze", _lib.ptr(mel32), _lib.ptr(W), _lib.ptr(bias), B, up.in_channels,
                  mel32.size(2), up.kernel_size[0], up.stride[0], m.n_group, L, w["Lp"], g["halo"],
                  _lib.ptr(w["Sh"]), _lib.ptr(w["Sl"]), _lib.current_stream())
        self._keep_up = (mel32, W, bias)

    def _wn(self, k, z, B, L, w, c_off, n_half, ph=None):
        m, g = self.m, self.geom()
        C, nl, ks = g["C"], g["nl"], g["ks"]
        fl = self.packed["flows"][k]
        st = _lib.current_stream()
        wn = m.WN[k]
        b_start = _f32c(wn.start.bias)
        self._keep_wn = [b_start]
        _lib.call("t2s_wg_start", _lib.ptr(z), _lib.ptr(fl["w_start"]), _lib.ptr(b_start), B, m.n_group, c_off, n_half,
                  C, L, w["Lp"], g["halo"], _lib.ptr(w["Xh"]), _lib.ptr(w["Xl"]), st)
        for i in range(nl):
            ly = fl["layers"][i]
            timed = self.gemm_events is not None and self._gemm_launch_no % self.gemm_event_stride == 0
            self._gemm_launch_no += 1
            if timed:
                e0, e1 = torch.cuda.Event(enable_timing=True), torch.cuda.Event(enable_timing=True)
                e0.record()
            if ph is not None:
                Mh, Ml, Fp, P, K2 = ph
                _lib.call("t2s_wg_in_melwin_gate_fold", _lib.ptr(ly["A1h"]), _lib.ptr(ly["A1l"]), _lib.ptr(ly["Ach"]),
                          _lib.ptr(ly["Acl"]), _lib.ptr(ly["b1c"]), _lib.ptr(w["Xh"]), _lib.ptr(w["Xl"]), _lib.ptr(Mh), _lib.ptr(Ml),
                          _lib.ptr(w["Ah"]), _lib.ptr(w["Al"]), _lib.ptr(ly["fold_A"]), _lib.ptr(w["fold_acc"]),
                          1 if i == 0 else 0, B, C, K2, ks, 2 ** i, L, w["Lp"], g["halo"], g["Mpad1"], P, Fp, st)
            elif self.use_fold:
                _lib.call("t2s_wg_in_cond_gate_fold", _lib.ptr(ly["A1h"]), _lib.ptr(ly["A1l"]), _lib.ptr(ly["b1"]),
                          _lib.ptr(w["Xh"]), _lib.ptr(w["Xl"]), _lib.ptr(w["Sh"]), _lib.ptr(w["Sl"]),
                          _lib.ptr(w["Ah"]), _lib.ptr(w["Al"]), _lib.ptr(ly["fold_A"]), _lib.ptr(w["fold_acc"]),
                          1 if i == 0 else 0, B, C, g["n_cond"], ks, 2 ** i, L, w["Lp"], g["halo"], g["Mpad1"], st)
            else:
                _lib.call("t2s_wg_in_cond_gate", _lib.ptr(ly["A1h"]), _lib.ptr(ly["A1l"]), _lib.ptr(ly["b1"]),
                          _lib.ptr(w["Xh"]), _lib.ptr(w["Xl"]), _lib.ptr(w["Sh"]), _lib.ptr(w["Sl"]),
                          _lib.ptr(w["Ah"]), _lib.ptr(w["Al"]), B, C, g["n_cond"], ks, 2 ** i, L, w["Lp"], g["halo"],
                          g["Mpad1"], st)
            if timed:
                e1.record()
                self.gemm_events.append((e0, e1))
            n_res = C if i < nl - 1 else 0
            if self.use_fold:
                if n_res:
                    _lib.call("t2s_wg_res_only", _lib.ptr(ly["A2h"]), _lib.ptr(ly["A2l"]), _lib.ptr(ly["b2"]),
                              _lib.ptr(w["Ah"]), _lib.ptr(w["Al"]), _lib.ptr(w["Xh"]), _lib.ptr(w["Xl"]), B, C, L, w["Lp"],
                              g["halo"], ly["Mpad2"], 1 if self.packed.get("res_pair8") else 0, st)
            else:
                _lib.call("t2s_wg_res_skip", _lib.ptr(ly["A2h"]), _lib.ptr(ly["A2l"]), _lib.ptr(ly["b2"]),
                          _lib.ptr(w["Ah"]), _lib.ptr(w["Al"]), _lib.ptr(w["Xh"]), _lib.ptr(w["Xl"]), _lib.ptr(w["skip"]),
                          B, C, n_res, 1 if i == 0 else 0, L, w["Lp"], g["halo"], ly["Mpad2"], st)

    def wn_forward(self, k, audio, spect):
        m = self.m
        self._check_inputs(audio, spect)
        dev = audio.device
        B, n_in, L = audio.shape
        c_off, n_rem, n_half = self._flow_geom(k)
        g = self.geom()
        if n_in != n_half or spect.size(1) != g["n_cond"] or spect.size(2) != L:
            raise ValueError("WN[%d] takes audio [B, %d, L] and spect [B, %d, L]" % (k, n_half, g["n_cond"]))
        self.pack_weights(dev, force=False, res_pair8=self.use_fold)
        w = self.workspace(B, L, dev)
        st = _lib.current_stream()
        spect32 = _f32c(spect)
        _lib.call("t2s_f32_to_planes", _lib.ptr(spect32), B, g["n_cond"], L, w["Lp"], g["halo"], _lib.ptr(w["Sh"]), _lib.ptr(w["Sl"]), st)
        z = torch.zeros(B, m.n_group, L, dtype=torch.float32, device=dev)
        z[:, c_off:c_off + n_half] = audio.detach().to(torch.float32)
        self._wn(k, z, B, L, w, c_off, n_half)
        wn_out = torch.empty(B, 2 * n_half, L, dtype=torch.float32, device=dev)
        if self.use_fold:
            w2 = dict(w)
            w2["wn_out"] = wn_out
            self._end(k, z, None, B, L, w2, c_off, n_half, reverse=False)
        else:
            self._end(k, z, None, B, L, w, c_off, n_half, reverse=False, wn_out=wn_out)
        self._keep_wnf = (spect32, z)
        return wn_out.to(audio.dtype)

    def _end(self, k, z, log_s, B, L, w, c_off, n_half, reverse, wn_out=None, skip=None):
        m, g = self.m, self.geom()
        wn = m.WN[k]
        w_end, b_end = _f32c(wn.end.weight), _f32c(wn.end.bias)
        self._keep_end = (w_end, b_end)
        if self.use_fold and wn_out is None and skip is None:
            fl = self.packed["flows"][k]
            _lib.call("t2s_wg_end_fold_affine", _lib.ptr(w["fold_acc"]), w["fold_acc"].size(0), _lib.ptr(fl["bes"]),
                      g["nl"], _lib.ptr(b_end), _lib.ptr(z), _lib.ptr(log_s), _lib.ptr(w.get("wn_out")), B, m.n_group, c_off,
                      n_half, L, 1 if reverse else 0, _lib.current_stream())
            return
        _lib.call("t2s_wg_end_affine", _lib.ptr(w["skip"] if skip is None else skip), _lib.ptr(w_end), _lib.ptr(b_end),
                  _lib.ptr(z), _lib.ptr(log_s), _lib.ptr(wn_out), B, m.n_group, c_off, n_half, g["C"], L, w["Lp"], g["halo"], 1 if reverse else 0,
                  _lib.current_stream())

    def _flow_geom(self, k):
        m = self.m
        c_off = m.n_early_size * (k // m.n_early_every)
        n_rem = m.n_group - c_off
        return c_off, n_rem, n_rem // 2

    def forward(self, mel, audio):
        m = self.m
        self._check_inputs(mel, audio)
        dev = audio.device
        B, T = audio.shape
        G = m.n_group
        L = T // G
        up = m.upsample
        if (mel.size(2) - 1) * up.stride[0] + up.kernel_size[0] < T:
            raise AssertionError("upsampled spectrogram shorter than audio (reference glow.py:216)")
        w = self.workspace(B, L, dev)
        main = torch.cuda.current_stream(dev)
        side = self.side_stream if getattr(self, "side_stream", None) is not None else torch.cuda.Stream(device=dev)
        self.side_stream = side
        audio32 = _f32c(audio)
        z = torch.empty(B, G, L, dtype=torch.float32, device=dev)
        log_s_list, log_det_list = [], []
        log_det = torch.empty(m.n_flows, dtype=torch.float32, device=dev)
        Ws = [_f32c(m.convinv[k].conv.weight) for k in range(m.n_flows)]
        keep = list(Ws)
        use_val = m.n_flows <= 16
        jobs = torch.tensor([[Ws[k].data_ptr(), log_det.data_ptr() + 4 * k, 0, self._flow_geom(k)[1]]
                             for k in range(m.n_flows)], dtype=torch.int64)
        if not use_val:
            jobs = jobs.to(dev)
        keep.append(jobs)
        side.wait_stream(main)
        with torch.cuda.stream(side):
            st2 = _lib.current_stream()
            _lib.call("t2s_wg_audio_squeeze", _lib.ptr(audio32), _lib.ptr(z), B, T, G, L, 0, st2)
            self._upsample(mel, B, L, w)
            ev_inputs = torch.cuda.Event()
            ev_inputs.record()
            if use_val:
                _lib.call("t2s_small_logdet_inv_batch_host", ctypes.c_void_p(jobs.data_ptr()), m.n_flows, float(B * L), st2)
            else:
                _lib.call("t2s_small_logdet_inv_batch", _lib.ptr(jobs), m.n_flows, float(B * L), st2)
        pack_s = self.pack_stream if getattr(self, "pack_stream", None) is not None else torch.cuda.Stream(device=dev)
        self.pack_stream = pack_s
        pack_events = []
        pack_s.wait_stream(main)
        with torch.cuda.stream(pack_s):
            self.pack_weights(dev, force=True, flow_events=pack_events, res_pair8=self.use_fold)
        main.wait_event(ev_inputs)
        st = _lib.current_stream()
        for k in range(m.n_flows):
            main.wait_event(pack_events[k])
            c_off, n_rem, n_half = self._flow_geom(k)
            Wk = Ws[k]
            _lib.call("t2s_wg_convinv", _lib.ptr(z), _lib.ptr(Wk), B, G, c_off, n_rem, L, st)
            self._wn(k, z, B, L, w, c_off, n_half)
            log_s = torch.empty(B, n_half, L, dtype=torch.float32, device=dev)
            self._end(k, z, log_s, B, L, w, c_off, n_half, reverse=False)
            log_s_list.append(log_s)
            log_det_list.append(log_det[k])
        main.wait_stream(side)
        self._keep_fwd = (audio32, keep)
        return z, log_s_list, log_det_list

    def infer(self, mel, sigma, noise):
        m = self.m
        self._check_inputs(mel)
        dev = mel.device
        B, _, frames = mel.shape
        G = m.n_group
        up = m.upsample
        T = (frames - 1) * up.stride[0] + up.kernel_size[0] - (up.kernel_size[0] - up.stride[0])
        L = T // G
        self.pack_weights(dev, force=False, res_pair8=self.use_fold)
        w = self.workspace(B, L, dev)
        st = _lib.current_stream()
        cg = self.compose_geom()
        C = self.geom()["C"]
        ph = None
        if cg is not None and _lib.load().t2s_wg_gate_tile_rows(B, C, L) == 256:
            P, nlag, K2 = cg
            self.compose_cond(dev)
            Fp = -(-frames // 256) * 256
            key = ("melwin", B, Fp, str(dev))
            mw = self.ws.get(key)
            if mw is None:
                mw = (torch.zeros(B, K2 // 32, Fp, 32, dtype=torch.bfloat16, device=dev),
                      torch.zeros(B, K2 // 32, Fp, 32, dtype=torch.bfloat16, device=dev))
                self.ws[key] = mw
            mel32 = _f32c(mel)
            _lib.call("t2s_wg_melwin_planes", _lib.ptr(mel32), B, mel32.size(1), frames, nlag, Fp, _lib.ptr(mw[0]), _lib.ptr(mw[1]), st)
            self._keep_up = (mel32,)
            ph = (mw[0], mw[1], Fp, P, K2)
        else:
            self._upsample(mel, B, L, w)
        z = torch.empty(B, G, L, dtype=torch.float32, device=dev)
        n_rem_final = m.n_remaining_channels
        early_ks = [k for k in reversed(range(m.n_flows)) if k % m.n_early_every == 0 and k > 0]
        if noise is None:
            noise_final = torch.randn(B, n_rem_final, L, dtype=torch.float32, device=dev)
            noise_early = [torch.randn(B, m.n_early_size, L, dtype=torch.float32, device=dev) for _ in early_ks]
        else:
            noise_final, noise_early = noise
        z[:, G - n_rem_final:] = sigma * noise_final.to(dev, torch.float32)
        for k, ne in zip(early_ks, noise_early):
            c_off = m.n_early_size * (k // m.n_early_every)
            z[:, c_off - m.n_early_size:c_off] = sigma * ne.to(dev, torch.float32)
        for k in reversed(range(m.n_flows)):
            c_off, n_rem, n_half = self._flow_geom(k)
            fl = self.packed["flows"][k]
            if fl["w_inv"] is None:
                Wk = _f32c(m.convinv[k].conv.weight)
                fl["w_inv"] = torch.empty(n_rem, n_rem, dtype=torch.float32, device=dev)
                _lib.call("t2s_small_logdet_inv", _lib.ptr(Wk), n_rem, 1.0, None, _lib.ptr(fl["w_inv"]), st)
                fl["_Wk"] = Wk
            self._wn(k, z, B, L, w, c_off, n_half, ph=ph)
            self._end(k, z, None, B, L, w, c_off, n_half, reverse=True)
            _lib.call("t2s_wg_convinv", _lib.ptr(z), _lib.ptr(fl["w_inv"]), B, G, c_off, n_rem, L, st)
        audio = torch.empty(B, L * G, dtype=torch.float32, device=dev)
        _lib.call("t2s_wg_audio_squeeze", _lib.ptr(audio), _lib.ptr(z), B, L * G, G, L, 1, st)
        return audio


class WaveGlow(torch.nn.Module):

    def __init__(self, n_mel_channels, n_flows, n_group, n_early_every, n_early_size, WN_config):
        super().__init__()
        self.upsample = torch.nn.ConvTranspose1d(n_mel_channels, n_mel_channels, 1024, stride=256)
        assert n_group % 2 == 0
        self.n_flows = n_flows
        self.n_group = n_group
        self.n_early_every = n_early_every
        self.n_early_size = n_early_size
        self.WN = torch.nn.ModuleList()
        self.convinv = torch.nn.ModuleList()
        n_half = n_group // 2
        n_remaining_channels = n_group
        for k in range(n_flows):
            if k % self.n_early_every == 0 and k > 0:
                n_half = n_half - self.n_early_size // 2
                n_remaining_channels = n_remaining_channels - self.n_early_size
            self.convinv.append(Invertible1x1Conv(n_remaining_channels))
            self.WN.append(WN(n_half, n_mel_channels * n_group, **WN_config))
        self.n_remaining_channels = n_remaining_channels
        self.__dict__["_engine"] = None
        self._adopt()

    def _adopt(self):
        import weakref
        for k, wn_k in enumerate(self.WN):
            wn_k.__dict__["_owner"] = weakref.ref(self)
            wn_k.__dict__["_flow"] = k

    def __setstate__(self, state):
        super().__setstate__(state)
        if "_engine" not in self.__dict__:
            self.__dict__["_engine"] = None
        self._adopt()

    def _eng(self):
        if self.__dict__.get("_engine") is None:
            self.__dict__["_engine"] = _Engine(self)
        return self.__dict__["_engine"]

    def __getstate__(self):
        d = self.__dict__.copy()
        d["_engine"] = None
        return d

    def forward(self, forward_input):
        spect, audio = forward_input
        f16 = _lib.operand_format() == 1
        if torch.is_grad_enabled() and any(p.requires_grad for p in self.parameters()):
            if f16:
                raise _lib.T2SError("the fp16-operand diagnostic build runs the no-grad forward / infer only: gradient planes "
                                    "underflow fp16 (use the shipped library for training)")
            from .glow_autograd import waveglow_forward_with_grad
            return waveglow_forward_with_grad(self, spect, audio)
        out = self._eng().forward(spect, audio)
        if f16:
            self._refuse_overflow(out[0])
        return out

    @staticmethod
    def _refuse_overflow(t):
        import os
        if os.environ.get("T2S_F16_GUARD", "1") == "0":
            return
        if not bool(torch.isfinite(t).all()):
            raise _lib.T2SError("fp16 operand planes overflowed (|x| > 65504 somewhere in the flow): result refused; "
                                "use the shipped split-bf16 library for this checkpoint / input")

    def infer(self, spect, sigma=1.0, noise=None):
        with torch.no_grad():
            out = self._eng().infer(spect, float(sigma), noise)
        if _lib.operand_format() == 1:
            self._refuse_overflow(out)
        return out.to(spect.dtype) if spect.dtype in (torch.float16, torch.bfloat16) else out

    @staticmethod
    def remove_weightnorm(model):
        waveglow = model
        for wn in waveglow.WN:
            wn.start = torch.nn.utils.remove_weight_norm(wn.start)
            wn.in_layers = remove(wn.in_layers)
            wn.cond_layers = remove(wn.cond_layers)
            wn.res_skip_layers = remove(wn.res_skip_layers)
        if waveglow.__dict__.get("_engine") is not None:
            waveglow.__dict__["_engine"].packed_key = None
        return waveglow


def remove(conv_list):
    new_conv_list = torch.nn.ModuleList()
    for old_conv in conv_list:
        new_conv_list.append(torch.nn.utils.remove_weight_norm(old_conv))
    return new_conv_list
```

### text2speech_amd/planes.py

```python
import torch

from . import _lib


def split_bf16(x):
    hi = x.to(torch.bfloat16)
    lo = (x - hi.to(torch.float32)).to(torch.bfloat16)
    return hi, lo


def to_planes(x, halo, Lp=None):
    B, C, L = x.shape
    if Lp is None:
        Lp = _lib.plane_rows(L, halo)
    nc = -(-C // 32)
    xp = torch.zeros(B, nc * 32, L, dtype=torch.float32, device=x.device)
    xp[:, :C] = x
    xp = xp.view(B, nc, 32, L).permute(0, 1, 3, 2)
    hi, lo = split_bf16(xp)
    ph = torch.zeros(B, nc, Lp, 32, dtype=torch.bfloat16, device=x.device)
    pl = torch.zeros_like(ph)
    ph[:, :, halo:halo + L] = hi
    pl[:, :, halo:halo + L] = lo
    return ph, pl


def from_planes(ph, pl, C, L, halo):
    B, nc = ph.shape[:2]
    v = ph[:, :, halo:halo + L].to(torch.float32) + pl[:, :, halo:halo + L].to(torch.float32)
    return v.permute(0, 1, 3, 2).reshape(B, nc * 32, L)[:, :C].contiguous()


def from_f32_planes(p, C, L, halo):
    B, nc = p.shape[:2]
    return p[:, :, halo:halo + L].permute(0, 1, 3, 2).reshape(B, nc * 32, L)[:, :C].contiguous()
```

Measured before the change: 7.440 million audio samples/s.

## Fold WN start conv into first layer's input conv via windowed audio

Precomposes the start 1x1 conv (with its bias) into the first WN layer's dilated input conv weights, so layer 0 reads a small windowed audio/ones tensor (taps x (n_half+1) columns) instead of the full C-channel start output. To keep precision with bf16x3 it encodes residual split terms as extra K columns (2 or 4 window chunks). It removes most of the K dimension for layer 0's gate GEMM, at the cost of extra weight packing and a more complex precision scheme. It is gated by use_fold and an environment flag, and is skipped when the mel-window composed conditioning path is active.

```diff
diff --git a/include/t2s_hip.h b/include/t2s_hip.h
--- a/include/t2s_hip.h
+++ b/include/t2s_hip.h
@@ -83,6 +83,15 @@
                              const void* S_hi, const void* S_lo, void* acts_hi, void* acts_lo, const void* fold_A,
                              float* fold_acc, int fold_init, int B, int C, int n_cond, int taps, int dilation, int L,
                              int Lp, int halo, int Mpad, void* stream);
+int t2s_wg_start_window(const float* z, const float* w, const float* bias, int B, int n_group, int c_off, int n_half, int C,
+                        int L, int Lp, int halo, void* X_hi, void* X_lo, int taps, int win_chunks, void* W_hi, void* W_lo,
+                        void* stream);
+int t2s_wg_startfold_weights(const float* v_in, const float* g_in, const float* w_start, const float* b_start, int C, int n_half,
+                             int taps, int Mpad, int win_chunks, void* A_hi, void* A_lo, void* stream);
+int t2s_wg_in_win_gate_fold(const void* A_hi, const void* A_lo, const float* bias, const void* W_hi, const void* W_lo,
+                            const void* S_hi, const void* S_lo, void* acts_hi, void* acts_lo, const void* fold_A,
+                            float* fold_acc, int fold_init, int B, int C, int n_cond, int win_chunks, int L, int Lp, int halo,
+                            int Mpad, void* stream);
 int t2s_wg_upsample_basis(const float* W, const float* bias, int n_mel, int ksize, int stride, int n_group, int Lp, int halo,
                           void* U_hi, void* U_lo, void* stream);
 int t2s_wg_compose_cond(const float* tmp, const float* bias_in, int rows, int Mpad, int P, int K2, long ld, void* A2_hi,
diff --git a/text2speech_amd/_lib.py b/text2speech_amd/_lib.py
--- a/text2speech_amd/_lib.py
+++ b/text2speech_amd/_lib.py
@@ -33,6 +33,9 @@
                         c_int, c_int, c_vp],
     "t2s_wg_endfold_weights": [c_vp, c_int, c_int, c_vp],
     "t2s_wg_in_cond_gate_fold": [c_vp] * 11 + [c_int] * 10 + [c_vp],
+    "t2s_wg_start_window": [c_vp, c_vp, c_vp] + [c_int] * 8 + [c_vp, c_vp, c_int, c_int, c_vp, c_vp, c_vp],
+    "t2s_wg_startfold_weights": [c_vp] * 4 + [c_int] * 5 + [c_vp, c_vp, c_vp],
+    "t2s_wg_in_win_gate_fold": [c_vp] * 11 + [c_int] * 9 + [c_vp],
     "t2s_wg_gate_fold_slots": [c_int, c_int, c_int],
     "t2s_wg_gate_tile_rows": [c_int, c_int, c_int],
     "t2s_wg_upsample_basis": [c_vp, c_vp] + [c_int] * 6 + [c_vp, c_vp, c_vp],
diff --git a/text2speech_amd/csrc/t2s_api.hip b/text2speech_amd/csrc/t2s_api.hip
--- a/text2speech_amd/csrc/t2s_api.hip
+++ b/text2speech_amd/csrc/t2s_api.hip
@@ -144,6 +144,32 @@
 
 static int check_planes(const void* a, const void* b) { return a && b && aligned16(a) && aligned16(b); }
 
+static bool win_chunks_ok(int taps, int n_half, int win_chunks) {
+    if (taps <= 0 || !(taps & 1) || n_half <= 0 || (win_chunks != 2 && win_chunks != 4)) return false;
+    return (4 / win_chunks) * taps * (n_half + 1) <= 32;
+}
+
+int t2s_wg_start_window(const float* z, const float* w, const float* bias, int B, int n_group, int c_off, int n_half, int C,
+                        int L, int Lp, int halo, void* X_hi, void* X_lo, int taps, int win_chunks, void* W_hi, void* W_lo,
+                        void* stream) {
+    if (!z || !w || !bias || !check_planes(X_hi, X_lo) || !check_planes(W_hi, W_lo)) return T2S_EINVAL;
+    if (B <= 0 || L <= 0 || C <= 0 || n_half <= 0 || n_half > 8 || c_off < 0 || c_off + n_half > n_group) return T2S_EINVAL;
+    if (!win_chunks_ok(taps, n_half, win_chunks) || cdiv(C, 32) < win_chunks || Lp < t2s_plane_rows(L, halo)) return T2S_EINVAL;
+    T2S_CHECK_HIP(t2s_launch_start(z, w, bias, B, n_group, c_off, n_half, C, L, Lp, halo, (u16*)X_hi, (u16*)X_lo,
+                                   (hipStream_t)stream, taps, win_chunks, (u16*)W_hi, (u16*)W_lo));
+    return T2S_OK;
+}
+
+int t2s_wg_startfold_weights(const float* v_in, const float* g_in, const float* w_start, const float* b_start, int C, int n_half,
+                             int taps, int Mpad, int win_chunks, void* A_hi, void* A_lo, void* stream) {
+    if (!v_in || !w_start || !b_start || !check_planes(A_hi, A_lo)) return T2S_EINVAL;
+    if (C <= 0 || !win_chunks_ok(taps, n_half, win_chunks)) return T2S_EINVAL;
+    if (Mpad % 256 || Mpad < cdiv(C, 128) * 256 || (size_t)C * (n_half + 1) * sizeof(float) > 60 * 1024) return T2S_EINVAL;
+    T2S_CHECK_HIP(t2s_launch_startfold_weights(v_in, g_in, w_start, b_start, C, n_half, taps, Mpad, win_chunks, (u16*)A_hi, (u16*)A_lo,
+                                               (hipStream_t)stream));
+    return T2S_OK;
+}
+
 int t2s_wg_in_cond_gate(const void* A_hi, const void* A_lo, const float* bias, const void* X_hi, const void* X_lo,
                         const void* S_hi, const void* S_lo, void* acts_hi, void* acts_lo, int B, int C, int n_cond,
                         int taps, int dilation, int L, int Lp, int halo, int Mpad, void* stream) {
@@ -232,6 +258,34 @@
     a.xc = cdiv(C, 32); a.sc = cdiv(n_cond, 32); a.oc = cdiv(C, 32);
     a.taps = taps; a.dil = dilation;
     a.nk_x = taps * a.xc; a.nk = a.nk_x + a.sc;
+    a.Mpad = Mpad; a.Lp = Lp; a.halo = halo; a.L = L; a.B = B;
+    const int rows = gate_tile_rows(B, C, L);
+    a.n_mtiles = cdiv(C, rows / 2); a.n_ttiles = cdiv(L, 256);
+    a.C = C;
+    T2S_CHECK_HIP(t2s_launch_conv_gemm(a, EPI_GATE, (hipStream_t)stream, rows));
+    return T2S_OK;
+}
+
+int t2s_wg_in_win_gate_fold(const void* A_hi, const void* A_lo, const float* bias, const void* W_hi, const void* W_lo,
+                            const void* S_hi, const void* S_lo, void* acts_hi, void* acts_lo, const void* fold_A,
+                            float* fold_acc, int fold_init, int B, int C, int n_cond, int win_chunks, int L, int Lp, int halo,
+                            int Mpad, void* stream) {
+    if (!check_planes(A_hi, A_lo) || !check_planes(W_hi, W_lo) || !check_planes(S_hi, S_lo) || !check_planes(acts_hi, acts_lo) ||
+        !bias)
+        return T2S_EINVAL;
+    if (!fold_A || !fold_acc || !aligned16(fold_A) || C % 16) return T2S_EINVAL;
+    if (B <= 0 || L <= 0 || C <= 0 || n_cond <= 0 || halo < 0 || Lp != t2s_plane_rows(L, halo)) return T2S_EINVAL;
+    if (Mpad % 256 || Mpad < cdiv(C, 128) * 256 || !aligned16(bias) || (win_chunks != 2 && win_chunks != 4)) return T2S_EINVAL;
+    ConvGemmArgs a;
+    memset(&a, 0, sizeof(a));
+    a.A_hi = (const u16*)A_hi; a.A_lo = (const u16*)A_lo;
+    a.X_hi = (const u16*)W_hi; a.X_lo = (const u16*)W_lo;
+    a.S_hi = (const u16*)S_hi; a.S_lo = (const u16*)S_lo;
+    a.bias = bias; a.O_hi = (u16*)acts_hi; a.O_lo = (u16*)acts_lo;
+    a.fold_A = (const u16*)fold_A; a.fold_acc = fold_acc; a.fold_init = fold_init;
+    a.xc = win_chunks; a.sc = cdiv(n_cond, 32); a.oc = cdiv(C, 32);
+    a.taps = 1; a.dil = 1;
+    a.nk_x = win_chunks; a.nk = win_chunks + a.sc;
     a.Mpad = Mpad; a.Lp = Lp; a.halo = halo; a.L = L; a.B = B;
     const int rows = gate_tile_rows(B, C, L);
     a.n_mtiles = cdiv(C, rows / 2); a.n_ttiles = cdiv(L, 256);
diff --git a/text2speech_amd/csrc/t2s_kernels.h b/text2speech_amd/csrc/t2s_kernels.h
--- a/text2speech_amd/csrc/t2s_kernels.h
+++ b/text2speech_amd/csrc/t2s_kernels.h
@@ -124,7 +124,10 @@
 hipError_t t2s_launch_small_logdet_inv(const float* W, int n, float scale, float* logdet_out, float* inv_out,
                                        hipStream_t stream);
 hipError_t t2s_launch_start(const float* z, const float* w, const float* bias, int B, int n_group, int c_off,
-                            int n_half, int C, int L, int Lp, int halo, u16* X_hi, u16* X_lo, hipStream_t stream);
+                            int n_half, int C, int L, int Lp, int halo, u16* X_hi, u16* X_lo, hipStream_t stream,
+                            int taps = 0, int nwc = 0, u16* W_hi = nullptr, u16* W_lo = nullptr);
+hipError_t t2s_launch_startfold_weights(const float* v, const float* g, const float* w_start, const float* b_start, int C,
+                                        int n_half, int taps, int Mpad, int nwc, u16* A_hi, u16* A_lo, hipStream_t stream);
 struct EndFoldJob {
     const float* w_end;
     const float* v_skip;
diff --git a/text2speech_amd/csrc/waveglow_ops.hip b/text2speech_amd/csrc/waveglow_ops.hip
--- a/text2speech_amd/csrc/waveglow_ops.hip
+++ b/text2speech_amd/csrc/waveglow_ops.hip
@@ -682,9 +682,22 @@
 }
 
 #define START_TT 8
+static __device__ __forceinline__ void start_fold_term(float x, int set, bool is_weight, u16& hi, u16& lo) {
+    u16 h, l;
+    split_bf16(x, h, l);
+    hi = h;
+    lo = l;
+    if (set == (is_weight ? 1 : 2)) {
+        split_bf16(x - join_bf16(h, l), hi, lo);
+    } else if (set == 3) {
+        hi = l;
+        lo = 0;
+    }
+}
 __global__ __launch_bounds__(256) void start_kernel(const float* __restrict__ z, const float* __restrict__ w,
                                                     const float* __restrict__ bias, int G, int c_off, int nh, int C,
-                                                    int L, int Lp, int halo, u16* X_hi, u16* X_lo) {
+                                                    int L, int Lp, int halo, u16* X_hi, u16* X_lo, int taps, int nwc,
+                                                    u16* W_hi, u16* W_lo) {
     const int tid = threadIdx.x;
     const int q = tid & 3;
     const int tbase = blockIdx.x * (64 * START_TT) + (tid >> 2);
@@ -725,12 +738,38 @@
         *(uint4*)(X_hi + (row0 + t) * 32 + q * 8) = ph;
         *(uint4*)(X_lo + (row0 + t) * 32 + q * 8) = pl;
     }
+    if (W_hi == nullptr || chunk >= nwc) return;
+    const int nw = nh + 1, ncol = taps * nw, spc = 4 / nwc;
+    const size_t wrow0 = ((size_t)b * nwc + chunk) * Lp + halo;
+    for (int it = 0; it < START_TT; ++it) {
+        const int t = tbase + it * 64;
+        if (t >= L) break;
+        u16 hi[8], lo[8];
+#pragma unroll
+        for (int e = 0; e < 8; ++e) {
+            const int col = q * 8 + e;
+            const int sidx = col / ncol, c = col - sidx * ncol;
+            const int tap = c / nw, j = c - tap * nw;
+            const int tt = t + tap - (taps >> 1);
+            float v = 0.f;
+            if (sidx < spc && tt >= 0 && tt < L) v = j < nh ? z[((size_t)b * G + c_off + j) * L + tt] : 1.0f;
+            start_fold_term(v, chunk * spc + sidx, false, hi[e], lo[e]);
+        }
+        uint4 ph, pl;
+        ph.x = hi[0] | ((uint32_t)hi[1] << 16); ph.y = hi[2] | ((uint32_t)hi[3] << 16);
+        ph.z = hi[4] | ((uint32_t)hi[5] << 16); ph.w = hi[6] | ((uint32_t)hi[7] << 16);
+        pl.x = lo[0] | ((uint32_t)lo[1] << 16); pl.y = lo[2] | ((uint32_t)lo[3] << 16);
+        pl.z = lo[4] | ((uint32_t)lo[5] << 16); pl.w = lo[6] | ((uint32_t)lo[7] << 16);
+        *(uint4*)(W_hi + (wrow0 + t) * 32 + q * 8) = ph;
+        *(uint4*)(W_lo + (wrow0 + t) * 32 + q * 8) = pl;
+    }
 }
 hipError_t t2s_launch_start(const float* z, const float* w, const float* bias, int B, int n_group, int c_off,
-                            int n_half, int C, int L, int Lp, int halo, u16* X_hi, u16* X_lo, hipStream_t stream) {
+                            int n_half, int C, int L, int Lp, int halo, u16* X_hi, u16* X_lo, hipStream_t stream,
+                            int taps, int nwc, u16* W_hi, u16* W_lo) {
     dim3 grid((L + 64 * START_TT - 1) / (64 * START_TT), (C + 31) / 32, B);
     hipLaunchKernelGGL(start_kernel, grid, dim3(256), 0, stream, z, w, bias, n_group, c_off, n_half, C, L, Lp, halo,
-                       X_hi, X_lo);
+                       X_hi, X_lo, taps, nwc, W_hi, W_lo);
     return hipGetLastError();
 }
 
@@ -844,6 +883,55 @@
     return hipGetLastError();
 }
 
+__global__ __launch_bounds__(256) void startfold_weights_kernel(const float* __restrict__ v, const float* __restrict__ g,
+                                                                const float* __restrict__ w_start,
+                                                                const float* __restrict__ b_start, int C, int nh, int Kt,
+                                                                int Mpad, int nwc, u16* A_hi, u16* A_lo) {
+    extern __shared__ float s_wb[];
+    const int tid = threadIdx.x, r = tid >> 5, col = tid & 31;
+    const int nw = nh + 1, n = C * Kt, O = 2 * C;
+    for (int i = tid; i < C * nw; i += 256) {
+        const int c = i / nw, j = i - c * nw;
+        s_wb[i] = j < nh ? w_start[c * nh + j] : b_start[c];
+    }
+    const int o = blockIdx.x * 8 + r;
+    const bool row_ok = o < O;
+    const float* vrow = v + (size_t)(row_ok ? o : 0) * n;
+    float scale = 1.0f;
+    if (g) {
+        float ss = 0.f;
+        for (int i = col; i < n; i += 32) ss += vrow[i] * vrow[i];
+        ss = sum16(ss);
+        ss += __shfl_xor(ss, 16, 64);
+        scale = g[row_ok ? o : 0] / sqrtf(ss);
+    }
+    __syncthreads();
+    if (!row_ok) return;
+    const int ncol = Kt * nw, spc = 4 / nwc;
+    const int sidx = col / ncol, lc = col - sidx * ncol;
+    float acc = 0.f;
+    if (sidx < spc) {
+        const int tap = lc / nw, j = lc - tap * nw;
+#pragma unroll 8
+        for (int c = 0; c < C; ++c) acc += vrow[c * Kt + tap] * s_wb[c * nw + j];
+    }
+    const int gate = o >= C;
+    const int ch = gate ? o - C : o;
+    const int p = (ch >> 7) * 256 + ((ch >> 6) & 1) * 128 + (((ch >> 4) & 3) * 2 + gate) * 16 + (ch & 15);
+    for (int wc = 0; wc < nwc; ++wc) {
+        u16 h, l;
+        start_fold_term(acc * scale, wc * spc + sidx, true, h, l);
+        A_hi[((size_t)wc * Mpad + p) * 32 + col] = h;
+        A_lo[((size_t)wc * Mpad + p) * 32 + col] = l;
+    }
+}
+hipError_t t2s_launch_startfold_weights(const float* v, const float* g, const float* w_start, const float* b_start, int C,
+                                        int n_half, int taps, int Mpad, int nwc, u16* A_hi, u16* A_lo, hipStream_t stream) {
+    hipLaunchKernelGGL(startfold_weights_kernel, dim3((2 * C + 7) / 8), dim3(256), (size_t)C * (n_half + 1) * sizeof(float),
+                       stream, v, g, w_start, b_start, C, n_half, taps, Mpad, nwc, A_hi, A_lo);
+    return hipGetLastError();
+}
+
 __global__ void end_fold_affine_kernel(const float* __restrict__ fold_acc, int nslots, const float* __restrict__ bes,
                                        int n_layers, const float* __restrict__ b_end, float* z, float* log_s, float* wn_out,
                                        int B, int G, int c_off, int nh, int L, int reverse) {
diff --git a/text2speech_amd/glow.py b/text2speech_amd/glow.py
--- a/text2speech_amd/glow.py
+++ b/text2speech_amd/glow.py
@@ -170,14 +170,23 @@
         halo = -(-((2 ** (nl - 1)) * (ks // 2)) // 32) * 32
         g = dict(C=C, nl=nl, ks=ks, n_cond=n_cond, Cpad=-(-C // 32) * 32, Spad=-(-n_cond // 32) * 32,
                  halo=halo, Mpad1=-(-C // 128) * 256)
+        g["ncol0"] = ks * (m.n_group // 2 + 1)
+        g["nwc"] = 2 if 2 * g["ncol0"] <= 32 else 4
         g["nk1"] = ks * g["Cpad"] // 32 + g["Spad"] // 32
         g["nk2"] = g["Cpad"] // 32
         return g
 
-    def pack_weights(self, device, force=True, flow_events=None, res_pair8=False):
+    def start_fold_on(self):
+        g = self.geom()
+        if not self.use_fold or os.environ.get("T2S_START_FOLD", "1") == "0" or g["C"] % 16 or self.compose_geom() is not None:
+            return False
+        return g["ncol0"] <= 32 and g["Cpad"] // 32 >= g["nwc"]
+
+    def pack_weights(self, device, force=True, flow_events=None, res_pair8=False, start_fold=False):
         m = self.m
         res_pair8 = bool(res_pair8) and self.geom()["C"] % 32 == 0
-        key = tuple(p._version for p in m.parameters()) + (str(device), res_pair8)
+        start_fold = bool(start_fold)
+        key = tuple(p._version for p in m.parameters()) + (str(device), res_pair8, start_fold)
         if not force and self.packed is not None and self.packed_key == key:
             return self.packed
         g = self.geom()
@@ -204,13 +213,17 @@
                         fold_A=torch.zeros(-(-C // 128) * 8192, dtype=torch.bfloat16, device=device)))
                 flows.append(dict(layers=layers, n_half=n_half, bes=torch.zeros(nl, 8, dtype=torch.float32, device=device),
                                   w_start=torch.empty(C, n_half, dtype=torch.float32, device=device),
+                                  A0h=torch.zeros(g["nwc"] + g["Spad"] // 32, g["Mpad1"], 32, dtype=torch.bfloat16, device=device),
+                                  A0l=torch.zeros(g["nwc"] + g["Spad"] // 32, g["Mpad1"], 32, dtype=torch.bfloat16, device=device),
                                   w_inv=None))
             self.packed = dict(flows=flows, device=device)
         srcs = []
         specs = []
+        in0 = []
         for k in range(m.n_flows):
             wn = m.WN[k]
             fl = self.packed["flows"][k]
+            specs.append([])
             for i in range(nl):
                 ly = fl["layers"][i]
                 v, gg = _vg(wn.in_layers[i])
@@ -220,28 +233,34 @@
                      _f32c(vc), None if gc is None else _f32c(gc),
                      _f32c(vr), None if gr is None else _f32c(gr), _f32c(wn.res_skip_layers[i].bias)]
                 srcs += t
-                specs.append((t[0], t[1], t[2], t[3], ly["A1h"], ly["A1l"], ly["b1"], 2 * C, C, ks, 1, C, g["Mpad1"], 0, g["Cpad"],
-                              ly["s_in"]))
-                specs.append((t[4], t[5], None, None, ly["A1h"], ly["A1l"], None, 2 * C, g["n_cond"], 1, 1, C, g["Mpad1"],
-                              ks * g["Cpad"], g["Spad"], ly["s_cond"]))
+                if i == 0:
+                    in0.append((t[0], t[1]))
+                if i == 0 and start_fold:
+                    specs[k].append((t[4], t[5], t[2], t[3], fl["A0h"], fl["A0l"], ly["b1"], 2 * C, g["n_cond"], 1, 1, C,
+                                     g["Mpad1"], 32 * g["nwc"], g["Spad"], ly["s_cond"]))
+                else:
+                    specs[k].append((t[0], t[1], t[2], t[3], ly["A1h"], ly["A1l"], ly["b1"], 2 * C, C, ks, 1, C, g["Mpad1"], 0,
+                                     g["Cpad"], ly["s_in"]))
+                    specs[k].append((t[4], t[5], None, None, ly["A1h"], ly["A1l"], None, 2 * C, g["n_cond"], 1, 1, C, g["Mpad1"],
+                                     ks * g["Cpad"], g["Spad"], ly["s_cond"]))
                 p8 = res_pair8 and i < nl - 1
-                specs.append((t[6], t[7], t[8], None, ly["A2h"], ly["A2l"], ly["b2"], t[6].size(0), C, 1, 2 if p8 else 0,
-                              C if p8 else 0, ly["Mpad2"], 0, g["Cpad"], ly["s_rs"]))
-        ptr_key = tuple(0 if t is None else t.data_ptr() for t in srcs) + (res_pair8,)
-        jpf = 3 * nl
+                specs[k].append((t[6], t[7], t[8], None, ly["A2h"], ly["A2l"], ly["b2"], t[6].size(0), C, 1, 2 if p8 else 0,
+                                 C if p8 else 0, ly["Mpad2"], 0, g["Cpad"], ly["s_rs"]))
+        ptr_key = tuple(0 if t is None else t.data_ptr() for t in srcs) + (res_pair8, start_fold)
         if self.packed.get("job_key") != ptr_key:
-            rows, flow_rows, row_start = [], [], 0
+            rows, flow_rows, flow_jobs = [], [], []
             dp = lambda t: 0 if t is None else t.data_ptr()
-            for n, (v, gg, b1, b2, Ah, Al, bo, O, Cin, Kt, perm, Cg, Mpad, koff, Cin_pad, so) in enumerate(specs):
-                if n % jpf == 0 and n:
-                    flow_rows.append(row_start)
-                    row_start = 0
-                rows.append([dp(v), dp(gg), dp(b1), dp(b2), dp(Ah), dp(Al), dp(bo), row_start,
-                             O, Cin, Kt, perm, Cg, Mpad, koff, Cin_pad, 0, 0, dp(so)])
-                row_start += -(-O // 16)
-            flow_rows.append(row_start)
+            for fspecs in specs:
+                row_start = 0
+                flow_jobs.append((len(rows), len(fspecs)))
+                for (v, gg, b1, b2, Ah, Al, bo, O, Cin, Kt, perm, Cg, Mpad, koff, Cin_pad, so) in fspecs:
+                    rows.append([dp(v), dp(gg), dp(b1), dp(b2), dp(Ah), dp(Al), dp(bo), row_start,
+                                 O, Cin, Kt, perm, Cg, Mpad, koff, Cin_pad, 0, 0, dp(so)])
+                    row_start += -(-O // 16)
+                flow_rows.append(row_start)
             self.packed["jobs"] = torch.tensor(rows, dtype=torch.int64).to(device)
             self.packed["flow_rows"] = flow_rows
+            self.packed["flow_jobs"] = flow_jobs
             self.packed["job_key"] = ptr_key
         fsrc = []
         for k in range(m.n_flows):
@@ -266,12 +285,18 @@
         for k in range(m.n_flows):
             wn = m.WN[k]
             fl = self.packed["flows"][k]
-            _lib.call("t2s_pack_conv_weight_table", _lib.c_vp(jobs_ptr + k * jpf * 19 * 8), jpf, self.packed["flow_rows"][k], st)
+            j0, nj = self.packed["flow_jobs"][k]
+            _lib.call("t2s_pack_conv_weight_table", _lib.c_vp(jobs_ptr + j0 * 19 * 8), nj, self.packed["flow_rows"][k], st)
             _lib.call("t2s_wg_endfold_weights", _lib.c_vp(fold_ptr + k * nl * 8 * 8), nl, C, st)
             v, gg = _vg(wn.start)
             v, gg = _f32c(v), (None if gg is None else _f32c(gg))
             starts += [v, gg]
             _lib.call("t2s_weightnorm_small", _lib.ptr(v), _lib.ptr(gg), C, fl["n_half"], _lib.ptr(fl["w_start"]), st)
+            if start_fold:
+                b_start = _f32c(wn.start.bias)
+                starts.append(b_start)
+                _lib.call("t2s_wg_startfold_weights", _lib.ptr(in0[k][0]), _lib.ptr(in0[k][1]), _lib.ptr(fl["w_start"]),
+                          _lib.ptr(b_start), C, fl["n_half"], ks, g["Mpad1"], g["nwc"], _lib.ptr(fl["A0h"]), _lib.ptr(fl["A0l"]), st)
             fl["w_inv"] = None
             if flow_events is not None:
                 ev = torch.cuda.Event()
@@ -280,6 +305,7 @@
         keep = srcs + [t for tup in fsrc for t in tup[:3]] + starts
         self.packed_key = key
         self.packed["res_pair8"] = res_pair8
+        self.packed["start_fold"] = start_fold
         self._keep = keep
         return self.packed
 
@@ -340,6 +366,7 @@
                      Xh=torch.zeros(B, xc, Lp, 32, **bf), Xl=torch.zeros(B, xc, Lp, 32, **bf),
                      Ah=torch.zeros(B, xc, Lp, 32, **bf), Al=torch.zeros(B, xc, Lp, 32, **bf),
                      Sh=torch.zeros(B, sc, Lp, 32, **bf), Sl=torch.zeros(B, sc, Lp, 32, **bf),
+                     Wh=torch.zeros(B, g["nwc"], Lp, 32, **bf), Wl=torch.zeros(B, g["nwc"], Lp, 32, **bf),
                      skip=torch.zeros(B, xc, Lp, 32, dtype=torch.float32, device=device),
                      fold_acc=torch.zeros(_lib.load().t2s_wg_gate_fold_slots(B, g["C"], L), B, 8, L, dtype=torch.float32,
                                           device=device))
@@ -370,16 +397,28 @@
         wn = m.WN[k]
         b_start = _f32c(wn.start.bias)
         self._keep_wn = [b_start]
-        _lib.call("t2s_wg_start", _lib.ptr(z), _lib.ptr(fl["w_start"]), _lib.ptr(b_start), B, m.n_group, c_off, n_half,
-                  C, L, w["Lp"], g["halo"], _lib.ptr(w["Xh"]), _lib.ptr(w["Xl"]), st)
+        sf = bool(self.packed.get("start_fold")) and self.use_fold and ph is None
+        if sf:
+            _lib.call("t2s_wg_start_window", _lib.ptr(z), _lib.ptr(fl["w_start"]), _lib.ptr(b_start), B, m.n_group, c_off, n_half,
+                      C, L, w["Lp"], g["halo"], _lib.ptr(w["Xh"]), _lib.ptr(w["Xl"]), ks, g["nwc"], _lib.ptr(w["Wh"]), _lib.ptr(w["Wl"]), st)
+        else:
+            _lib.call("t2s_wg_start", _lib.ptr(z), _lib.ptr(fl["w_start"]), _lib.ptr(b_start), B, m.n_group, c_off, n_half,
+                      C, L, w["Lp"], g["halo"], _lib.ptr(w["Xh"]), _lib.ptr(w["Xl"]), st)
         for i in range(nl):
             ly = fl["layers"][i]
-            timed = self.gemm_events is not None and self._gemm_launch_no % self.gemm_event_stride == 0
-            self._gemm_launch_no += 1
+            full_k = not (sf and i == 0)
+            timed = full_k and self.gemm_events is not None and self._gemm_launch_no % self.gemm_event_stride == 0
+            if full_k:
+                self._gemm_launch_no += 1
             if timed:
                 e0, e1 = torch.cuda.Event(enable_timing=True), torch.cuda.Event(enable_timing=True)
                 e0.record()
-            if ph is not None:
+            if not full_k:
+                _lib.call("t2s_wg_in_win_gate_fold", _lib.ptr(fl["A0h"]), _lib.ptr(fl["A0l"]), _lib.ptr(ly["b1"]),
+                          _lib.ptr(w["Wh"]), _lib.ptr(w["Wl"]), _lib.ptr(w["Sh"]), _lib.ptr(w["Sl"]),
+                          _lib.ptr(w["Ah"]), _lib.ptr(w["Al"]), _lib.ptr(ly["fold_A"]), _lib.ptr(w["fold_acc"]),
+                          1, B, C, g["n_cond"], g["nwc"], L, w["Lp"], g["halo"], g["Mpad1"], st)
+            elif ph is not None:
                 Mh, Ml, Fp, P, K2 = ph
                 _lib.call("t2s_wg_in_melwin_gate_fold", _lib.ptr(ly["A1h"]), _lib.ptr(ly["A1l"]), _lib.ptr(ly["Ach"]),
                           _lib.ptr(ly["Acl"]), _lib.ptr(ly["b1c"]), _lib.ptr(w["Xh"]), _lib.ptr(w["Xl"]), _lib.ptr(Mh), _lib.ptr(Ml),
@@ -418,7 +457,7 @@
         g = self.geom()
         if n_in != n_half or spect.size(1) != g["n_cond"] or spect.size(2) != L:
             raise ValueError("WN[%d] takes audio [B, %d, L] and spect [B, %d, L]" % (k, n_half, g["n_cond"]))
-        self.pack_weights(dev, force=False, res_pair8=self.use_fold)
+        self.pack_weights(dev, force=False, res_pair8=self.use_fold, start_fold=self.start_fold_on())
         w = self.workspace(B, L, dev)
         st = _lib.current_stream()
         spect32 = _f32c(spect)
@@ -499,7 +538,7 @@
         pack_events = []
         pack_s.wait_stream(main)
         with torch.cuda.stream(pack_s):
-            self.pack_weights(dev, force=True, flow_events=pack_events, res_pair8=self.use_fold)
+            self.pack_weights(dev, force=True, flow_events=pack_events, res_pair8=self.use_fold, start_fold=self.start_fold_on())
         main.wait_event(ev_inputs)
         st = _lib.current_stream()
         for k in range(m.n_flows):
@@ -525,7 +564,7 @@
         up = m.upsample
         T = (frames - 1) * up.stride[0] + up.kernel_size[0] - (up.kernel_size[0] - up.stride[0])
         L = T // G
-        self.pack_weights(dev, force=False, res_pair8=self.use_fold)
+        self.pack_weights(dev, force=False, res_pair8=self.use_fold, start_fold=self.start_fold_on())
         w = self.workspace(B, L, dev)
         st = _lib.current_stream()
         cg = self.compose_geom()
diff --git a/text2speech_amd/planes.py b/text2speech_amd/planes.py
--- a/text2speech_amd/planes.py
+++ b/text2speech_amd/planes.py
@@ -34,3 +34,32 @@
 def from_f32_planes(p, C, L, halo):
     B, nc = p.shape[:2]
     return p[:, :, halo:halo + L].permute(0, 1, 3, 2).reshape(B, nc * 32, L)[:, :C].contiguous()
+
+
+def start_window(a, taps):
+    B, nh, L = a.shape
+    x = torch.cat([a, torch.ones(B, 1, L, dtype=a.dtype, device=a.device)], 1)
+    xp = torch.nn.functional.pad(x, (taps // 2, taps // 2))
+    return torch.cat([xp[:, :, tap:tap + L] for tap in range(taps)], 1)
+
+
+def start_fold_matrix(w_in, w_start, b_start):
+    C = w_in.size(1)
+    wb = torch.cat([w_start.reshape(C, -1), b_start.reshape(C, 1)], 1)
+    return torch.einsum("mct,cj->mtj", w_in, wb).reshape(w_in.size(0), -1)
+
+
+def start_fold_sets(x, is_weight, nwc, axis):
+    h, l = split_bf16(x)
+    rh, rl = split_bf16(x - (h.to(torch.float32) + l.to(torch.float32)))
+    z = torch.zeros_like(l)
+    sets = [(h, l), (rh, rl) if is_weight else (h, l), (h, l) if is_weight else (rh, rl), (l, z)]
+    spc, ncol = 4 // nwc, x.size(axis)
+    shape = list(x.shape)
+    shape[axis] = 32 * nwc
+    hi, lo = torch.zeros(shape, dtype=torch.bfloat16, device=x.device), torch.zeros(shape, dtype=torch.bfloat16, device=x.device)
+    for s_, (a, b) in enumerate(sets):
+        c0 = (s_ // spc) * 32 + (s_ % spc) * ncol
+        hi.narrow(axis, c0, ncol).copy_(a)
+        lo.narrow(axis, c0, ncol).copy_(b)
+    return hi, lo
```

Result: faster. 7.772 million audio samples/s, median of 6 (+4.5%).
